# humanoid-path-planner/hpp-fcl

Hardware: AMD Instinct MI355X
Metric: narrow-phase queries/s (collision+distance) (higher is better)
Workload: dtype f32; 1 GPU; cfg3_convex32_distance_nesterov; request=distance, gather=none

## Files before the change

### hpp-fcl_amd/csrc/hfcl_dev.hpp

```cpp
#pragma once
#include <hip/hip_runtime.h>

#include <cstdint>
#include <cstring>
#include <type_traits>

#include "../../include/hppfcl_amd.h"
#include "hfcl_bvh.hpp"
#include "hfcl_bvh_shape.hpp"
#include "hfcl_pair.hpp"

using namespace hfcl;

#ifndef HFCL_WPE_GJK_W2
#define HFCL_WPE_GJK_W2 2
#endif
#ifndef HFCL_WPE_GJK
#define HFCL_WPE_GJK 3
#endif
#ifndef HFCL_WPE_GJK64
#define HFCL_WPE_GJK64 2
#endif
#ifndef HFCL_WPE_PRIM
#define HFCL_WPE_PRIM 2
#endif
#ifndef HFCL_WPE_EPA32
#define HFCL_WPE_EPA32 2
#endif
#ifndef HFCL_WPE_EPA64
#define HFCL_WPE_EPA64 1
#endif
#ifndef HFCL_WPE_BVH
#define HFCL_WPE_BVH 1
#endif

enum { B_CLOSED = 0, B_PRIM = 1, B_CC = 2, B_PC = 3, B_CP = 4, B_BVH = 5, B_UNSUPPORTED = 6, B_LARGE = 7, B_BVHSHAPE = 8, B_TRI = 9, B_COUNT = 10 };
constexpr int B_CURVED0 = B_COUNT + 4;
constexpr int CTR_SHAPE_TICKET = 2 * B_COUNT + 4, CTR_SHAPE_DEFER = 2 * B_COUNT + 5;
constexpr int CTR_DIST_SUSP = 2 * B_COUNT + 6;
constexpr int CTR_SHAPE_DIST_SUSP = 2 * B_COUNT + 7;
constexpr int CTR_DIST_TICKET = 2 * B_COUNT + 8;
constexpr int CTR_SHAPE_DIST_TICKET = 2 * B_COUNT + 9;
constexpr int CTR_EPA_CC_OVER = 2 * B_COUNT + 10;
constexpr int CTR_SHAPE_FINISH_OVER = 2 * B_COUNT + 11;
constexpr int CTR_SHAPE_DEFER_MARK = 2 * B_COUNT + 13;
constexpr int CTR_DIST_RERUN = 2 * B_COUNT + 14, CTR_SHAPE_DIST_RERUN = 2 * B_COUNT + 15;
constexpr int N_COUNTERS = 2 * B_COUNT + 16;

constexpr int K_CONVEX_LARGE = 21;

__host__ __device__ inline int bucket_of(int k1, int k2, bool distance_mode = false) {
  if (distance_mode && (k1 == K_TRIANGLE || k2 == K_TRIANGLE)) return B_UNSUPPORTED;
  const bool large = (k1 == K_CONVEX_LARGE) || (k2 == K_CONVEX_LARGE);
  if (k1 == K_CONVEX_LARGE) k1 = K_CONVEX;
  if (k2 == K_CONVEX_LARGE) k2 = K_CONVEX;
  if ((k1 == K_BVH) != (k2 == K_BVH)) {
    const int o = (k1 == K_BVH) ? k2 : k1;
    return (kind_is_prim(o) || o == K_CONVEX || kind_is_flat(o)) ? B_BVHSHAPE : B_UNSUPPORTED;
  }
  if ((k1 == K_TRIANGLE || k2 == K_TRIANGLE) && !kind_is_flat(k1) && !kind_is_flat(k2)) {
    const int o = (k1 == K_TRIANGLE) ? k2 : k1;
    return (o == K_TRIANGLE || kind_is_prim(o) || o == K_CONVEX) ? B_TRI : B_UNSUPPORTED;
  }
  const int c = pair_class(k1, k2);
  if (large && c == CLS_CONVEX) return B_LARGE;
  if (c == CLS_CLOSED) return B_CLOSED;
  if (c == CLS_PRIM_GJK) return B_PRIM;
  if (c == CLS_BVH) return B_BVH;
  if (c == CLS_CONVEX) {
    if (k1 == K_CONVEX && k2 == K_CONVEX) return B_CC;
    return (k1 == K_CONVEX) ? B_CP : B_PC;
  }
  return B_UNSUPPORTED;
}

template <typename T>
struct NbrEntry;
template <> struct alignas(16) NbrEntry<float> { float x, y, z; uint32_t id; };
template <> struct alignas(32) NbrEntry<double> { double x, y, z; uint32_t id; uint32_t pad_; };

template <typename T>
struct LibView {
  const DShape<T>* shapes;
  const T* verts;
  const uint8_t* kinds;
  uint32_t n_shapes;
  const uint32_t* graph_base;
  const uint32_t* graph_off;
  const NbrEntry<T>* graph_ent;
  uint32_t climb_min;
};
static constexpr uint32_t HFCL_NO_GRAPH = 0xFFFFFFFFu;
#ifndef HFCL_CLIMB_MIN
#define HFCL_CLIMB_MIN 512u
#endif
static constexpr int HFCL_WARM_STARTS = 14;
template <typename T>
struct HullGraph {
  const uint32_t* off;
  const NbrEntry<T>* ent;
};
template <typename T>
__device__ __forceinline__ HullGraph<T> hull_graph(const LibView<T>& lib, uint32_t shape_id, uint32_t num_points) {
  HullGraph<T> g{nullptr, nullptr};
  if (lib.graph_base == nullptr || num_points < lib.climb_min) return g;
  const uint32_t base = lib.graph_base[shape_id];
  if (base == HFCL_NO_GRAPH) return g;
  g.off = lib.graph_off + base;
  g.ent = lib.graph_ent;
  return g;
}

template <typename T> struct IO;
template <> struct IO<double> {
  const double* tf1;
  const double* tf2;
  hfcl_result* out;
  const hfcl_guess* gin;
  hfcl_guess* gout;
};
template <> struct IO<float> {
  const float* tf1;
  const float* tf2;
  hfcl_result_f32* out;
  const hfcl_guess* gin;
  hfcl_guess* gout;
};

template <typename T> using EpaItem = EpaSeed<T>;

struct Work {
  const uint32_t* shape1;
  const uint32_t* shape2;
  uint32_t n;
  uint32_t* lists;
  uint32_t* counts;
  void* epa_queue;
  void* epa_queue2;
  void* epa_v0;
  void* epa_resume;
  uint32_t resume_cap;
  void* shape_defer;
  uint32_t shape_defer_cap;
  uint32_t* shape_finish_over;
  void* shape_oq;
  void* epa_ready;
  void* epa_ready_g;
  uint32_t* epa_cc_over;
  uint32_t cc_resume_base, cc_resume_cap;
};
__host__ __device__ inline bool curved_pair(int k1, int k2) {
  return k1 == K_ELLIPSOID || k1 == K_CONE || k1 == K_CYLINDER || k2 == K_ELLIPSOID || k2 == K_CONE || k2 == K_CYLINDER;
}
struct BucketList {
  const uint32_t* base;
  uint32_t n, c0, cnt;
  __device__ __forceinline__ uint32_t operator[](uint32_t i) const { return i < c0 ? base[i] : base[n - 1u - (i - c0)]; }
};
__device__ __forceinline__ BucketList bucket_list(const Work& wk, int b) {
  const uint32_t c0 = wk.counts[b];
  return BucketList{wk.lists + size_t(b) * wk.n, wk.n, c0, c0 + wk.counts[B_CURVED0 + b]};
}
constexpr int32_t EPA_RESUME_FLAG = 0x100;
constexpr int32_t EPA_RESUME_SMALL = 0x200;

__device__ __forceinline__ Pose<double> load_pose(const double* base, uint32_t i) { return pose_from_abi<double>(base + 12 * size_t(i)); }
__device__ __forceinline__ void put_record(hfcl_result* dst, const hfcl_result& r) { *dst = r; }
__device__ __forceinline__ Pose<float> load_pose(const float* base, uint32_t i) { return pose_from_quat<float>(base + 7 * size_t(i)); }

__device__ __forceinline__ void store_record(const IO<double>& io, uint32_t pair, const PairOut<double>& o, bool contact,
                                             int nc) {
  hfcl_result r;
  r.distance = o.distance;
  r.normal[0] = o.normal.x; r.normal[1] = o.normal.y; r.normal[2] = o.normal.z;
  r.p1[0] = o.p1.x; r.p1[1] = o.p1.y; r.p1[2] = o.p1.z;
  r.p2[0] = o.p2.x; r.p2[1] = o.p2.y; r.p2[2] = o.p2.z;
  r.b1 = -1;
  r.b2 = -1;
  r.status = pack_status(o.gjk_status, o.epa_status, contact, o.gjk_iters, o.epa_iters);
  r.num_contacts = nc;
  put_record(&io.out[pair], r);
}
__device__ __forceinline__ void store_record(const IO<float>& io, uint32_t pair, const PairOut<float>& o, bool contact,
                                             int) {
  hfcl_result_f32 r;
  r.distance = o.distance;
  r.p1[0] = o.p1.x; r.p1[1] = o.p1.y; r.p1[2] = o.p1.z;
  r.p2[0] = o.p2.x; r.p2[1] = o.p2.y; r.p2[2] = o.p2.z;
  r.normal[0] = o.normal.x; r.normal[1] = o.normal.y; r.normal[2] = o.normal.z;
  r.status = pack_status(o.gjk_status, o.epa_status, contact, o.gjk_iters, o.epa_iters);
  io.out[pair] = r;
}
template <typename T>
__device__ __forceinline__ void write_out(const IO<T>& io, const QParams<T>& q, uint32_t pair, PairOut<T> o) {
  int nc;
  const bool contact = apply_query_semantics(q, o, nc);
  store_record(io, pair, o, contact, nc);
}

__device__ __forceinline__ void store_bvh_record(const IO<double>& io, uint32_t pair, const PairOut<double>& o, uint32_t nc,
                                                 int b1, int b2, bool overflow) {
  hfcl_result r;
  r.distance = o.distance;
  r.normal[0] = o.normal.x; r.normal[1] = o.normal.y; r.normal[2] = o.normal.z;
  r.p1[0] = o.p1.x; r.p1[1] = o.p1.y; r.p1[2] = o.p1.z;
  r.p2[0] = o.p2.x; r.p2[1] = o.p2.y; r.p2[2] = o.p2.z;
  r.b1 = b1;
  r.b2 = b2;
  r.status = (nc ? 128u : 0u) | (overflow ? 0xC0000000u : 0u);
  r.num_contacts = int(nc & 0x7FFFFFFFu);
  io.out[pair] = r;
}
__device__ __forceinline__ void store_bvh_record(const IO<float>& io, uint32_t pair, const PairOut<float>& o, uint32_t nc,
                                                 int, int, bool overflow) {
  hfcl_result_f32 r;
  r.distance = o.distance;
  r.p1[0] = o.p1.x; r.p1[1] = o.p1.y; r.p1[2] = o.p1.z;
  r.p2[0] = o.p2.x; r.p2[1] = o.p2.y; r.p2[2] = o.p2.z;
  r.normal[0] = o.normal.x; r.normal[1] = o.normal.y; r.normal[2] = o.normal.z;
  r.status = (nc ? 128u : 0u) | (overflow ? 0xC0000000u : 0u);
  io.out[pair] = r;
}

__device__ __forceinline__ void store_witness(const IO<double>& io, uint32_t pair, const V3<double>& p1, const V3<double>& p2, const V3<double>& n) {
  hfcl_result* r = &io.out[pair];
  r->normal[0] = n.x; r->normal[1] = n.y; r->normal[2] = n.z;
  r->p1[0] = p1.x; r->p1[1] = p1.y; r->p1[2] = p1.z;
  r->p2[0] = p2.x; r->p2[1] = p2.y; r->p2[2] = p2.z;
}
__device__ __forceinline__ void store_witness(const IO<float>& io, uint32_t pair, const V3<float>& p1, const V3<float>& p2, const V3<float>& n) {
  hfcl_result_f32* r = &io.out[pair];
  r->p1[0] = p1.x; r->p1[1] = p1.y; r->p1[2] = p1.z;
  r->p2[0] = p2.x; r->p2[1] = p2.y; r->p2[2] = p2.z;
// ... 504 lines not shown
```

### hpp-fcl_amd/csrc/hfcl_host.hip

```cpp
#include <algorithm>
#include <chrono>
#include <cstdio>
#include <cstdlib>
#include <cstring>
#include <condition_variable>
#include <map>
#include <mutex>
#include <thread>
#include <string>
#include <vector>

#include "hfcl_dev.hpp"
#include "hfcl_launch.hpp"
#include "hfcl_patch.hpp"
#include "hfcl_scene.hpp"

static thread_local std::string g_last_error;
static void set_error(const std::string& s) { g_last_error = s; }
void hfcl_internal_set_error(const char* msg) { g_last_error = msg ? msg : ""; }

#define HIP_TRY(expr)                                                                         \
  do {                                                                                        \
    hipError_t _e = (expr);                                                                   \
    if (_e != hipSuccess) {                                                                   \
      set_error(std::string(#expr) + ": " + hipGetErrorString(_e));                           \
      return HFCL_ERR_HIP;                                                                    \
    }                                                                                         \
  } while (0)

struct KernelTime {
  const char* name;
  hipEvent_t e0, e1;
  bool used;
};

struct hfcl_lib {
  int device = 0;
  size_t n_shapes = 0;
  std::vector<hfcl_shape> h_shapes;
  std::vector<uint8_t> h_kinds;
  DShape<double>* d_shapes64 = nullptr;
  DShape<float>* d_shapes32 = nullptr;
  double* d_verts64 = nullptr;
  float* d_verts32 = nullptr;
  uint8_t* d_kinds = nullptr;
  std::vector<double> h_verts;
  struct HostGraph { std::vector<uint32_t> off, ids; };
  std::map<uint32_t, HostGraph> h_graphs;
  bool graph_dirty = false;
  uint32_t* d_graph_base = nullptr;
  std::vector<void*> graph_retired;
  hipStream_t upload_stream = nullptr;
  uint32_t* d_graph_off = nullptr;
  NbrEntry<float>* d_graph_ent32 = nullptr;
  NbrEntry<double>* d_graph_ent64 = nullptr;
  uint32_t climb_min = HFCL_CLIMB_MIN;
  size_t ws_capacity = 0;
  size_t epa_capacity = 0;
  uint32_t* d_lists = nullptr;
  uint32_t* d_counts = nullptr;
  void* d_epa_queue = nullptr;
  void* d_epa_queue2 = nullptr;
  uint32_t* d_epa_cc_over = nullptr;
  hipStream_t aux = nullptr;
  hipStream_t mesh_st = nullptr;
  hipEvent_t ev_mesh_fork = nullptr, ev_mesh_join = nullptr;
  hipStream_t mesh_st2 = nullptr, mesh_aux = nullptr;
  bool ran_batch = false;
  hipEvent_t ev_mesh_fork2 = nullptr, ev_mesh_join2 = nullptr;
  BvhTask* d_bvh2_tasks = nullptr;
  void* d_bvh2_sums = nullptr;
  uint32_t* d_bvh2_susp = nullptr;
  uint32_t* d_bvh2_ctr = nullptr;
  size_t bvh2_split_n = 0, bvh2_split_cap = 0;
  uint32_t mesh_beside = 2;
  bool mesh_prio = false;
  hipStream_t gjk_st[3] = {nullptr, nullptr, nullptr};
  hipEvent_t gjk_fork = nullptr, gjk_join[3] = {nullptr, nullptr, nullptr};
  uint32_t epa_direct_max = 4096;
  uint32_t gjk_beside_max = 120000;
  hipStream_t walk_st[WALK_ROUNDS - 1] = {};
  hipEvent_t walk_fork[WALK_ROUNDS - 1] = {}, walk_join[WALK_ROUNDS - 1] = {};
  hipEvent_t ev_aux0 = nullptr, ev_aux1 = nullptr, ev_aux2 = nullptr, ev_aux3 = nullptr;
  void* d_epa_ready = nullptr;
  size_t epa_ready_capacity = 0;
  void* d_epa_ready_g = nullptr;
  size_t epa_ready_g_bytes = 0;
  bool epa_general_staged = false;
  size_t epa_general_staged_min = 32768;
  bool records_aside = true;
  bool epa64_two_streams = true;
  bool epa_cc_staged = true;
  size_t epa_cc_staged_min = 32768;
  void* d_epa_resume = nullptr;
  void* d_epa_v0 = nullptr;
  size_t resume_cap = 0;
  bool shape_finish_tiers = true;
  bool shape_finish_aside = true;
  void* d_shape_defer = nullptr;
  void* d_shape_oq = nullptr;
  size_t shape_defer_capacity = 0, shape_oq_capacity = 0;
  bool bvh_shape_lane = true;
  uint32_t shape_budget0 = 128, shape_budget = 96, shape_leaf_cost = 32, shape_levels = BVH_MAX_LEVELS;
  bool shape_coop = true;
  uint32_t bvh_cut_ticks = 0, shape_cut_ticks = 350000;
  uint32_t shape_budget0_coop = 16;
  bool bvh_coop = true;
  uint32_t bvh_budget0_coop = 0;
  uint32_t bvhd_budget = 64;
  uint32_t bvhd_pool = 1;
  uint32_t bvhd_pool_leaf_min = 24, bvhd_pool_starve = 32, bvhd_pool_part_min = 48;
  void* d_dist_susp = nullptr;
  size_t dist_susp_capacity = 0;
  uint32_t pool_rerun = 1;
  uint32_t shape_dist_pool = 1;
  uint32_t shape_dist_leaf_min = 48, shape_dist_starve = 16;
  uint32_t shape_dist_budget = 64;
  void* d_shape_dist_susp = nullptr;
  size_t shape_dist_susp_capacity = 0;
  static constexpr int PIPE_SLOTS = 6;
  struct Staging {
    uint32_t *d_s1 = nullptr, *d_s2 = nullptr;
    double *d_tf1 = nullptr, *d_tf2 = nullptr;
    double *d_qt1 = nullptr, *d_qt2 = nullptr;
    hfcl_result* d_out = nullptr;
    hfcl_guess *d_gin = nullptr, *d_gout = nullptr;
    hipEvent_t ev_in = nullptr, ev_in2 = nullptr, ev_done = nullptr;
    uint32_t* h_counts = nullptr;
    uint32_t* h_counts2 = nullptr;
    bool split = false;
  };
  Staging stage[PIPE_SLOTS];
  size_t st_capacity = 0;
  static constexpr size_t SMALL_MAX = 4096;
  char* h_pack = nullptr;
  char* d_pack = nullptr;
  uint32_t* h_pack_counts = nullptr;
  hipStream_t s_h2d = nullptr, s_h2d2 = nullptr, s_cmp = nullptr, s_d2h = nullptr;
  uint32_t acc_counts[N_COUNTERS] = {0};
  bool last_host = false;
  bool in_host_batch = false;
  size_t pipe_chunk = 0;
  uint32_t* counts_dst = nullptr;
  std::vector<KernelTime> timers;
  int split = 0;
  hfcl_lib* helper = nullptr;
  bool is_helper = false;
  bool last_split = false;
  hipStream_t side = nullptr;
  hipEvent_t ev_fork = nullptr, ev_join = nullptr;
  bool kernel_timing = true;
// ... 220 lines not shown
  lib->graph_dirty = true;
  std::vector<DShape<double>> s64(n_shapes);
  std::vector<DShape<float>> s32(n_shapes);
  std::vector<uint8_t> kinds(n_shapes);
  for (size_t i = 0; i < n_shapes; ++i) {
    const hfcl_shape& s = shapes[i];
    s64[i].kind = s.type;
    s64[i].num_points = s.num_points;
    s64[i].vertex_offset = s.vertex_offset;
    s64[i].bvh_index = s.bvh_index;
    s64[i].p0 = s.params[0];
    s64[i].p1 = s.params[1];
    s64[i].p2 = s.params[2];
    s64[i].p3 = s.params[3];
    s64[i].ssr = s.swept_sphere_radius;
    s32[i].kind = s.type;
    s32[i].num_points = s.num_points;
    s32[i].vertex_offset = s.vertex_offset;
    s32[i].bvh_index = s.bvh_index;
    s32[i].p0 = float(s.params[0]);
    s32[i].p1 = float(s.params[1]);
    s32[i].p2 = float(s.params[2]);
    s32[i].p3 = float(s.params[3]);
    s32[i].ssr = float(s.swept_sphere_radius);
    if (s.type == HFCL_GEOM_CONVEX && s.num_points > 0 && vertices &&
        size_t(s.vertex_offset) + s.num_points <= n_vertices) {
      double mn[3], mx[3];
      const double* v = vertices + 3 * size_t(s.vertex_offset);
      for (int k = 0; k < 3; ++k) mn[k] = mx[k] = v[k];
      for (uint32_t j = 1; j < s.num_points; ++j)
        for (int k = 0; k < 3; ++k) {
          mn[k] = std::min(mn[k], v[3 * size_t(j) + k]);
          mx[k] = std::max(mx[k], v[3 * size_t(j) + k]);
        }
      s64[i].p0 = (mn[0] + mx[0]) * 0.5; s64[i].p1 = (mn[1] + mx[1]) * 0.5; s64[i].p2 = (mn[2] + mx[2]) * 0.5;
      s32[i].p0 = float(s64[i].p0); s32[i].p1 = float(s64[i].p1); s32[i].p2 = float(s64[i].p2);
    }
    kinds[i] = uint8_t(s.type == HFCL_GEOM_CONVEX && s.num_points > (uint32_t)HULL_MAX ? K_CONVEX_LARGE : s.type);
  }
  {
    bool present[256] = {false};
    for (size_t i = 0; i < n_shapes; ++i) present[kinds[i]] = true;
    uint32_t mask = 1u << B_UNSUPPORTED;
    for (int a = 0; a < 256; ++a)
      if (present[a])
        for (int b = 0; b < 256; ++b)
          if (present[b]) mask |= 1u << bucket_of(a, b);
    lib->possible_buckets = mask;
    lib->has_curved = present[K_ELLIPSOID] || present[K_CONE] || present[K_CYLINDER];
    lib->has_flats = present[K_PLANE] || present[K_HALFSPACE];
  }
  lib->h_kinds = kinds;
  std::vector<float> v32(3 * n_vertices + 3);
  for (size_t i = 0; i < 3 * n_vertices; ++i) v32[i] = float(vertices[i]);
  hipFree(lib->d_shapes64); hipFree(lib->d_shapes32); hipFree(lib->d_kinds); hipFree(lib->d_verts64); hipFree(lib->d_verts32);
  lib->d_shapes64 = nullptr; lib->d_shapes32 = nullptr; lib->d_kinds = nullptr; lib->d_verts64 = nullptr; lib->d_verts32 = nullptr;
  bool ok = true;
  ok = ok && hipMalloc(&lib->d_shapes64, n_shapes * sizeof(DShape<double>)) == hipSuccess;
  ok = ok && hipMalloc(&lib->d_shapes32, n_shapes * sizeof(DShape<float>)) == hipSuccess;
  ok = ok && hipMalloc(&lib->d_kinds, n_shapes) == hipSuccess;
  ok = ok && hipMalloc(&lib->d_verts64, (3 * n_vertices + 3) * sizeof(double)) == hipSuccess;
  ok = ok && hipMalloc(&lib->d_verts32, (3 * n_vertices + 3) * sizeof(float)) == hipSuccess;
  if (ok) {
    ok = ok && hipMemcpy(lib->d_shapes64, s64.data(), n_shapes * sizeof(DShape<double>), hipMemcpyHostToDevice) == hipSuccess;
    ok = ok && hipMemcpy(lib->d_shapes32, s32.data(), n_shapes * sizeof(DShape<float>), hipMemcpyHostToDevice) == hipSuccess;
    ok = ok && hipMemcpy(lib->d_kinds, kinds.data(), n_shapes, hipMemcpyHostToDevice) == hipSuccess;
    if (n_vertices) {
      ok = ok && hipMemcpy(lib->d_verts64, vertices, 3 * n_vertices * sizeof(double), hipMemcpyHostToDevice) == hipSuccess;
      ok = ok && hipMemcpy(lib->d_verts32, v32.data(), 3 * n_vertices * sizeof(float), hipMemcpyHostToDevice) == hipSuccess;
    }
  }
  return ok;
}


static const char* const* option_keys() {
  static const char* const keys[] = {
      "closed_staged", "split", "epa_cc_staged", "epa_records_aside", "epa_general_staged", "shape_finish_tiers", "shape_finish_aside",
      "epa_general_staged_min", "epa64_two_streams", "epa_cc_staged_min", "pipe_chunk", "bvh_filter", "bvh_shape_lane", "shape_coop",
      "bvh_cut_ticks", "shape_cut_ticks", "bvh_coop", "bvhd_budget", "bvhd_pool", "shape_dist_pool", "pool_rerun", "bvh_walk_early_coop",
      "bvh_walk_rounds", "bvh_walk_order", "mesh_beside", "mesh_prio", "shape_walk", "shape_walk_sort", "shape_walk_budget", "shape_walk_min", "gjk_beside_max", "epa_direct_max", "bvh_walk_k", "bvh_walk_budget", "shape_dist_leaf_min", "shape_dist_starve", "bvhd_leaf_min", "bvhd_starve",
      "bvhd_part_min", "shape_dist_budget", "bvh_budget0_coop", "shape_budget0", "shape_budget", "shape_leaf_cost", "shape_levels",
      "climb_min", "bvh_budget", "bvh_budget0", "bvh_levels", "cvx_w", "epa_resume_slots", "bvh_task_slots", "bvh_force_wide",
      "pipe_trace", "scene_chunk", nullptr};
  return keys;
}
static int parse_list(const char* v, uint32_t* out, int first, int cap, uint32_t lo, uint32_t hi) {
  int k = first;
  for (const char* p = v; *p && k < cap; ++k) {
    const long long x = atoll(p);
    out[k] = uint32_t(std::min<long long>(std::max<long long>(x, lo), hi));
    while (*p && *p != ',') ++p;
    if (*p == ',') ++p;
  }
  return k - first;
}
static int apply_option(hfcl_lib* lib, const std::string& key, const char* v) {
  const long long i = atoll(v);
  const bool on = i != 0;
  auto u32 = [&](long long lo) { return uint32_t(std::min<long long>(std::max(i, lo), 0xFFFFFFFFll)); };
  if (key == "closed_staged") lib->closed_staged = on;
  else if (key == "split") lib->split = i >= 2 ? 2 : (i == 1 ? 1 : 0);
  else if (key == "epa_cc_staged") lib->epa_cc_staged = on;
  else if (key == "epa_records_aside") lib->records_aside = on;
  else if (key == "epa_general_staged") {
    if (on && !HFCL_KEEP_AB_FORMS) return HFCL_ERR_INVALID_ARGUMENT;
    lib->epa_general_staged = on;
  }
  else if (key == "shape_finish_tiers") lib->shape_finish_tiers = on;
  else if (key == "shape_finish_aside") lib->shape_finish_aside = on;
  else if (key == "epa_general_staged_min") lib->epa_general_staged_min = size_t(std::max(0ll, i));
  else if (key == "epa64_two_streams") lib->epa64_two_streams = on;
  else if (key == "epa_cc_staged_min") lib->epa_cc_staged_min = size_t(std::max(0ll, i));
  else if (key == "pipe_chunk") lib->pipe_chunk = strtoull(v, nullptr, 10);
  else if (key == "bvh_filter") {
    if (on && !HFCL_KEEP_AB_FORMS) return HFCL_ERR_INVALID_ARGUMENT;
    lib->bvh_filter = on;
  }
  else if (key == "bvh_shape_lane") lib->bvh_shape_lane = on;
  else if (key == "shape_coop") lib->shape_coop = on;
  else if (key == "bvh_cut_ticks") lib->bvh_cut_ticks = uint32_t(strtoul(v, nullptr, 10));
  else if (key == "shape_cut_ticks") lib->shape_cut_ticks = uint32_t(strtoul(v, nullptr, 10));
  else if (key == "bvh_coop") lib->bvh_coop = on;
  else if (key == "bvhd_budget") lib->bvhd_budget = u32(0);
  else if (key == "bvhd_pool") lib->bvhd_pool = u32(0);
  else if (key == "shape_dist_pool") lib->shape_dist_pool = u32(0);
  else if (key == "pool_rerun") lib->pool_rerun = u32(0);
  else if (key == "bvh_walk_early_coop") lib->walk_early_coop = on;
  else if (key == "bvh_walk_order") lib->walk_order = on;
  else if (key == "mesh_beside") lib->mesh_beside = u32(0);
  else if (key == "shape_walk") lib->shape_walk = on;
  else if (key == "mesh_prio") lib->mesh_prio = on;
  else if (key == "shape_walk_sort") lib->shape_walk_sort = on;
  else if (key == "shape_walk_budget") lib->shape_walk_budget = u32(0);
  else if (key == "shape_walk_min") lib->shape_walk_min = u32(0);
  else if (key == "gjk_beside_max") lib->gjk_beside_max = u32(0);
  else if (key == "epa_direct_max") lib->epa_direct_max = u32(0);
  else if (key == "bvh_walk_rounds") { lib->walk_rounds = uint32_t(std::min<long long>(std::max(0ll, i), WALK_ROUNDS)); lib->walk_auto = false; }
  else if (key == "bvh_walk_k") { parse_list(v, lib->walk_k, 0, WALK_ROUNDS, 1u, uint32_t(WALK_K)); lib->walk_auto = false; }
  else if (key == "bvh_walk_budget") parse_list(v, lib->walk_budget, 1, WALK_ROUNDS, 0u, 0xFFFFFFFFu);
  else if (key == "shape_dist_leaf_min") lib->shape_dist_leaf_min = u32(1);
  else if (key == "shape_dist_starve") lib->shape_dist_starve = u32(1);
  else if (key == "bvhd_leaf_min") lib->bvhd_pool_leaf_min = u32(1);
  else if (key == "bvhd_starve") lib->bvhd_pool_starve = u32(1);
  else if (key == "bvhd_part_min") lib->bvhd_pool_part_min = u32(0);
  else if (key == "shape_dist_budget") lib->shape_dist_budget = u32(0);
  else if (key == "bvh_budget0_coop") lib->bvh_budget0_coop = u32(1);
  else if (key == "shape_budget0") lib->shape_budget0 = lib->shape_budget0_coop = uint32_t(i);
  else if (key == "shape_budget") lib->shape_budget = uint32_t(i);
  else if (key == "shape_leaf_cost") lib->shape_leaf_cost = u32(1);
  else if (key == "shape_levels") lib->shape_levels = uint32_t(std::min<long long>(std::max(1ll, i), BVH_MAX_LEVELS));
  else if (key == "climb_min") lib->climb_min = u32(0);
  else if (key == "bvh_budget") { lib->bvh_budget = lib->bvh_budget0 = u32(0); lib->bvh_auto = false; }
  else if (key == "bvh_budget0") { lib->bvh_budget0 = u32(0); lib->bvh_auto = false; }
  else if (key == "bvh_levels") { lib->bvh_levels = uint32_t(std::min<long long>(BVH_MAX_LEVELS, std::max(1ll, i))); lib->bvh_auto = false; }
  else if (key == "cvx_w") {
    if (i == 0 || i == 2 || i == 4 || i == 8 || i == 16 || i == 32 || i == 64) lib->cvx_w = int(i);
    else return HFCL_ERR_INVALID_ARGUMENT;
  }
  else if (key == "epa_resume_slots") lib->epa_resume_slots = size_t(std::max(0ll, i));
  else if (key == "bvh_task_slots") lib->bvh_task_slots = size_t(std::max(0ll, i));
  else if (key == "bvh_force_wide") lib->bvh_force_wide = on;
  else if (key == "pipe_trace") lib->pipe_trace = on;
  else if (key == "scene_chunk") {
    if (i < 0 || i > 0xFFFFFFF0ll) return HFCL_ERR_INVALID_ARGUMENT;
    lib->scene_chunk = size_t(i);
  }
  else return HFCL_ERR_INVALID_ARGUMENT;
  return HFCL_OK;
}

hfcl_lib* hfcl_lib_create(const hfcl_shape* shapes, size_t n_shapes, const double* vertices, size_t n_vertices,
                          int device) {
  if (ensure_device(device) != HFCL_OK) return nullptr;
  if (!validate_shapes("hfcl_lib_create", shapes, n_shapes, vertices, n_vertices)) return nullptr;
  hfcl_lib* lib = new hfcl_lib();
  lib->device = device;
  bool ok = upload_shapes(lib, shapes, n_shapes, vertices, n_vertices);
  ok = ok && hipMalloc(&lib->d_counts, N_COUNTERS * sizeof(uint32_t)) == hipSuccess;
  ok = ok && hipHostMalloc((void**)&lib->h_counts, N_COUNTERS * sizeof(uint32_t), hipHostMallocDefault) == hipSuccess;
  if (ok) memset(lib->h_counts, 0, N_COUNTERS * sizeof(uint32_t));
  if (!ok) {
    set_error("hfcl_lib_create: HIP allocation/copy failed");
    hfcl_lib_destroy(lib);
    return nullptr;
  }
  hipDeviceProp_t prop;
  if (hipGetDeviceProperties(&prop, device) == hipSuccess) lib->n_cus = prop.multiProcessorCount;
  if (hipMalloc(&lib->d_epa_v0, size_t(lib->n_cus) * 16 * (64 / EPA_WE2) * EPA_MAX_VERTS * sizeof(Quad<double>)) != hipSuccess) {
    set_error("hfcl_lib_create: HIP allocation failed");
    hfcl_lib_destroy(lib);
    return nullptr;
  }
  for (const char* const* k = option_keys(); *k; ++k) {
    std::string name = "HFCL_";
    for (const char* c = *k; *c; ++c) name.push_back(char(toupper(static_cast<unsigned char>(*c))));
    if (const char* v = getenv(name.c_str())) apply_option(lib, *k, v);
  }
  return lib;
}

void hfcl_lib_destroy(hfcl_lib* lib) {
  if (!lib) return;
  hipSetDevice(lib->device);
  hipDeviceSynchronize();
  if (lib->helper) hfcl_lib_destroy(lib->helper);
  if (!lib->is_helper) free_retired_graphs(lib);
  if (lib->upload_stream) hipStreamDestroy(lib->upload_stream);
  if (lib->side) hipStreamDestroy(lib->side);
  if (lib->ev_fork) hipEventDestroy(lib->ev_fork);
  if (lib->ev_join) hipEventDestroy(lib->ev_join);
  if (!lib->is_helper) {
    hipFree(lib->d_shapes64);
    hipFree(lib->d_shapes32);
    hipFree(lib->d_kinds);
    hipFree(lib->d_verts64);
    hipFree(lib->d_verts32);
    hipFree(lib->d_graph_base);
    hipFree(lib->d_graph_off);
    hipFree(lib->d_graph_ent32);
    hipFree(lib->d_graph_ent64);
  }
  hipFree(lib->d_counts);
  if (lib->h_counts) hipHostFree(lib->h_counts);
  hipFree(lib->d_patch_ws);
  hipFree(lib->d_patch_lists);
  hipFree(lib->d_patch_counts);
  if (lib->patch_st) hipStreamDestroy(lib->patch_st);
  {
    hfcl_lib::SceneWs& w = lib->scene;
    hipFree(w.d_s1); hipFree(w.d_s2); hipFree(w.d_tf1); hipFree(w.d_tf2); hipFree(w.d_gin); hipFree(w.d_partials); hipFree(w.d_table); hipFree(w.d_summary);
    for (int k = 0; k < 2; ++k) {
      hipFree(w.d_rec[k]);
      hipFree(w.d_gout[k]);
      if (w.ev_done[k]) hipEventDestroy(w.ev_done[k]);
      if (w.ev_copied[k]) hipEventDestroy(w.ev_copied[k]);
    }
    if (w.s_cmp) hipStreamDestroy(w.s_cmp);
    if (w.s_copy) hipStreamDestroy(w.s_copy);
    if (w.h_counts) hipHostFree(w.h_counts);
    for (hipEvent_t e : w.ev_counts)
      if (e) hipEventDestroy(e);
  }
  hipFree(lib->d_lists);
  hipFree(lib->d_epa_queue);
  hipFree(lib->d_epa_queue2);
  hipFree(lib->d_epa_ready);
  hipFree(lib->d_epa_ready_g);
  hipFree(lib->d_epa_cc_over);
  if (lib->mesh_st) hipStreamDestroy(lib->mesh_st);
  if (lib->mesh_st2) hipStreamDestroy(lib->mesh_st2);
  if (lib->mesh_aux) hipStreamDestroy(lib->mesh_aux);
  for (hipEvent_t e : {lib->ev_mesh_fork, lib->ev_mesh_join, lib->ev_mesh_fork2, lib->ev_mesh_join2})
    if (e) hipEventDestroy(e);
  hipFree(lib->d_bvh2_tasks); hipFree(lib->d_bvh2_sums); hipFree(lib->d_bvh2_susp); hipFree(lib->d_bvh2_ctr);
  for (int k = 0; k < 3; ++k) {
    if (lib->gjk_st[k]) hipStreamDestroy(lib->gjk_st[k]);
    if (lib->gjk_join[k]) hipEventDestroy(lib->gjk_join[k]);
  }
  if (lib->gjk_fork) hipEventDestroy(lib->gjk_fork);
  for (int k = 0; k < WALK_ROUNDS - 1; ++k) {
    if (lib->walk_st[k]) hipStreamDestroy(lib->walk_st[k]);
    if (lib->walk_fork[k]) hipEventDestroy(lib->walk_fork[k]);
    if (lib->walk_join[k]) hipEventDestroy(lib->walk_join[k]);
  }
  if (lib->aux) hipStreamDestroy(lib->aux);
  if (lib->ev_aux0) hipEventDestroy(lib->ev_aux0);
  if (lib->ev_aux1) hipEventDestroy(lib->ev_aux1);
  if (lib->ev_aux2) hipEventDestroy(lib->ev_aux2);
  if (lib->ev_aux3) hipEventDestroy(lib->ev_aux3);
  hipFree(lib->d_epa_resume);
  hipFree(lib->d_epa_v0);
  hipFree(lib->d_shape_defer);
  hipFree(lib->d_shape_oq);
  hipFree(lib->d_dist_susp);
  hipFree(lib->d_shape_dist_susp);
  if (lib->h_pack) hipHostFree(lib->h_pack);
  if (lib->h_pack_counts) hipHostFree(lib->h_pack_counts);
  hipFree(lib->d_pack);
  for (auto& sg : lib->stage) {
    hipFree(sg.d_s1);
    hipFree(sg.d_s2);
    hipFree(sg.d_tf1);
    hipFree(sg.d_tf2);
    hipFree(sg.d_qt1);
    hipFree(sg.d_qt2);
    hipFree(sg.d_out);
    hipFree(sg.d_gin);
    hipFree(sg.d_gout);
    if (sg.ev_in) hipEventDestroy(sg.ev_in);
    if (sg.ev_done) hipEventDestroy(sg.ev_done);
    if (sg.ev_in2) hipEventDestroy(sg.ev_in2);
    if (sg.h_counts) hipHostFree(sg.h_counts);
    if (sg.h_counts2) hipHostFree(sg.h_counts2);
  }
  if (lib->s_h2d) hipStreamDestroy(lib->s_h2d);
  if (lib->s_h2d2) hipStreamDestroy(lib->s_h2d2);
  if (lib->s_cmp) hipStreamDestroy(lib->s_cmp);
  if (lib->s_d2h) hipStreamDestroy(lib->s_d2h);
  hipFree(lib->d_nodes64);
  hipFree(lib->d_nodes32);
  hipFree(lib->d_fnodes);
  hipFree(lib->d_rss64);
  hipFree(lib->d_rss32);
  hipFree(lib->d_dnodes64);
  hipFree(lib->d_dnodes32);
// ... 552 lines not shown
  for (int k = 0; k < 3; ++k) {
    lib->gjk_st[k] = s[k];
    lib->gjk_join[k] = ev[k];
  }
  lib->gjk_fork = ev[3];
  return HFCL_OK;
}
template <typename T, int M>
static int auto_cvx_w() {
  return (sizeof(T) == 8 && M == 0) ? 4 : 2;
}
template <typename T, int M>
static void launch_cvx_m(hfcl_lib* lib, const Work& wk, const LibView<T>& lv, const IO<T>& io, const QParams<T>& q,
                         hipStream_t st, size_t n) {
  const int w = lib->cvx_w ? lib->cvx_w : auto_cvx_w<T, M>();
  size_t b = (n + size_t(256 / w) - 1) / size_t(256 / w);
  if (b < 1) b = 1;
  if (b > size_t(lib->n_cus) * 16) b = size_t(lib->n_cus) * 16;
  launch_gjk_cvx<T>(M, w, q.guess_mode == HFCL_GUESS_BOUNDING_VOLUME, int(b), st, wk, lv, io, q);
}
template <typename T, class Next>
static void launch_cvx(hfcl_lib* lib, const Work& wk, const LibView<T>& lv, const IO<T>& io, const QParams<T>& q,
                       hipStream_t st, size_t& ti, size_t n, Next&& next_stream) {
  KernelTime* t = nullptr;
  auto tbeg = [&](const char* name) {
    if (!lib->kernel_timing) return;
    t = timer_slot(lib, ti++, name);
    hipEventRecord(t->e0, st);
  };
  auto tend = [&]() {
    if (lib->kernel_timing) hipEventRecord(t->e1, st);
  };
  if ((lib->possible_buckets >> B_CC) & 1u) {
    st = next_stream();
    tbeg("k_gjk_cvx<cc>");
    launch_cvx_m<T, 0>(lib, wk, lv, io, q, st, n);
    tend();
  }
  if ((lib->possible_buckets >> B_PC) & 1u) {
    st = next_stream();
    tbeg("k_gjk_cvx<pc>");
    launch_cvx_m<T, 1>(lib, wk, lv, io, q, st, n);
    tend();
  }
  if ((lib->possible_buckets >> B_CP) & 1u) {
    st = next_stream();
    tbeg("k_gjk_cvx<cp>");
    launch_cvx_m<T, 2>(lib, wk, lv, io, q, st, n);
    tend();
  }
}

template <typename T>
static int run_batch_one(hfcl_lib* lib, const uint32_t* d_s1, const uint32_t* d_s2, IO<T> io, size_t n, QParams<T> q,
                         hipStream_t st) {
  if (n == 0) return HFCL_OK;
  if (n > 0xFFFFFFF0ull) {
    set_error("batch too large (max 2^32-16 pairs per call)");
    return HFCL_ERR_LIMIT;
  }
  HIP_TRY(hipSetDevice(lib->device));
  const bool any_gjk_bucket = ((lib->possible_buckets >> B_PRIM) | (lib->possible_buckets >> B_CC) | (lib->possible_buckets >> B_PC) |
                               (lib->possible_buckets >> B_CP) | (lib->possible_buckets >> B_LARGE)) & 1u;
  int rc = ensure_workspace(lib, n, any_gjk_bucket && q.compute_penetration);
  if (rc) return rc;
  Work wk;
  wk.shape1 = d_s1;
  wk.shape2 = d_s2;
  wk.n = uint32_t(n);
  wk.lists = lib->d_lists;
  wk.counts = lib->d_counts;
  wk.epa_queue = lib->d_epa_queue;
  wk.epa_queue2 = lib->d_epa_queue2;
  wk.epa_resume = lib->d_epa_resume;
  wk.epa_v0 = lib->d_epa_v0;
  wk.resume_cap = uint32_t(std::min<size_t>(lib->resume_cap, 0xFFFFFFFFu));
  wk.shape_defer = nullptr;
  wk.shape_defer_cap = 0;
  wk.shape_finish_over = nullptr;
  wk.shape_oq = nullptr;
  wk.epa_ready = nullptr;
  wk.epa_ready_g = nullptr;
  wk.epa_cc_over = lib->d_epa_cc_over;
  wk.cc_resume_base = wk.resume_cap;
  {
    const size_t fslots = lib->resume_cap * std::max(epa_resume_stride<double>, epa_resume_stride<float>) / epa_resume_stride<float>;
    wk.cc_resume_cap = std::is_same<T, float>::value && fslots > lib->resume_cap ? uint32_t(std::min<size_t>(fslots - lib->resume_cap, lib->resume_cap)) : 0u;
  }
  LibView<T> lv;
  lv.shapes = std::is_same<T, double>::value ? (const DShape<T>*)lib->d_shapes64 : (const DShape<T>*)lib->d_shapes32;
  lv.verts = std::is_same<T, double>::value ? (const T*)lib->d_verts64 : (const T*)lib->d_verts32;
  lv.kinds = lib->d_kinds;
  lv.n_shapes = uint32_t(lib->n_shapes);
  lv.graph_base = lib->d_graph_base;
  lv.graph_off = lib->d_graph_off;
  lv.graph_ent = std::is_same<T, double>::value ? (const NbrEntry<T>*)lib->d_graph_ent64 : (const NbrEntry<T>*)lib->d_graph_ent32;
  lv.climb_min = lib->climb_min;

  for (auto& t : lib->timers) t.used = false;
  size_t ti = 0;
  const int max_blocks = lib->n_cus * 16;
  auto blocks_for = [&](size_t items, size_t per_block) {
    size_t b = (items + per_block - 1) / per_block;
    if (b < 1) b = 1;
    if (b > (size_t)max_blocks) b = max_blocks;
    return int(b);
  };
  KernelTime* t = nullptr;
  auto tbeg = [&](const char* name) {
    if (!lib->kernel_timing) return;
    t = timer_slot(lib, ti++, name);
    hipEventRecord(t->e0, st);
  };
  auto tend = [&]() {
    if (lib->kernel_timing) hipEventRecord(t->e1, st);
  };
  auto may = [&](int b) { return (lib->possible_buckets >> b) & 1u; };
  const bool any_gjk = may(B_PRIM) || may(B_CC) || may(B_PC) || may(B_CP) || may(B_LARGE);
  const bool bvg = q.guess_mode == HFCL_GUESS_BOUNDING_VOLUME;
  HIP_TRY(hipMemsetAsync(lib->d_counts, 0, N_COUNTERS * sizeof(uint32_t), st));
  tbeg("k_classify");
  launch_classify(blocks_for(n, CLS_BLOCK * 8), st, wk, lib->d_kinds, uint32_t(lib->n_shapes), q.mode != 1);
  tend();

  auto launch_solids = [&]() -> int {
    int kernels = 0;
    for (int b : {int(B_PRIM), int(B_CC), int(B_PC), int(B_CP), int(B_LARGE), int(B_TRI)}) kernels += may(b) ? 1 : 0;
    bool fan = lib->gjk_beside_max && n <= lib->gjk_beside_max && lib->h_meshes.empty() && kernels >= 3;
    if (fan && ensure_gjk_streams(lib) != HFCL_OK) fan = false;
    hipStream_t const caller = st;
    int fan_i = 0;
    uint32_t used = 0;
    if (fan) HIP_TRY(hipEventRecord(lib->gjk_fork, caller));
    auto next_stream = [&]() -> hipStream_t {
      if (!fan) return caller;
      const int k = fan_i;
      fan_i = (fan_i + 1) % 4;
      if (k && !(used & (1u << (k - 1)))) {
        used |= 1u << (k - 1);
        (void)hipStreamWaitEvent(lib->gjk_st[k - 1], lib->gjk_fork, 0);
      }
      return k ? lib->gjk_st[k - 1] : caller;
    };
    if (may(B_CLOSED)) {
      st = next_stream();
      tbeg("k_closed");
      launch_closed<T>(blocks_for(n, 256), st, wk, lv, io, q, lib->closed_staged);
      tend();
    }
    if (may(B_PRIM)) {
      st = next_stream();
      tbeg("k_gjk_prim");
      launch_gjk_prim<T>(blocks_for(n, 256), st, wk, lv, io, q, bvg);
      tend();
    }

    launch_cvx<T>(lib, wk, lv, io, q, caller, ti, n, next_stream);

    if (may(B_LARGE)) {
      st = next_stream();
      tbeg("k_gjk_large");
      launch_gjk_large<T>(blocks_for(n, 256 / LARGE_W), st, wk, lv, io, q, bvg);
      tend();
    }

    if (may(B_TRI)) {
      st = next_stream();
      tbeg("k_triangle");
      launch_triangle<T>(blocks_for(n / 8 + 1, 64 / BS_W), st, wk, lv, io, q);
      tend();
    }
    st = caller;
    for (int k = 0; k < 3; ++k)
      if (used & (1u << k)) {
        HIP_TRY(hipEventRecord(lib->gjk_join[k], lib->gjk_st[k]));
        HIP_TRY(hipStreamWaitEvent(caller, lib->gjk_join[k], 0));
      }
    return HFCL_OK;
  };
  bool meshes_on_own_stream = false;
  auto launch_meshes = [&]() -> int {
    if (!lib->h_meshes.empty() && (may(B_BVH) || may(B_BVHSHAPE))) {
      const hfcl_lib* owner = lib;
      for (const hfcl_shape& sh : owner->h_shapes)
        if (sh.type == HFCL_BV_OBBRSS && (sh.bvh_index < 0 || size_t(sh.bvh_index) >= owner->h_meshes.size())) {
          set_error("BVH shape with bvh_index " + std::to_string(sh.bvh_index) + " but only " + std::to_string(owner->h_meshes.size()) +
                    " BVHModel(s) registered (hfcl_lib_add_bvh)");
          return HFCL_ERR_INVALID_ARGUMENT;
        }
      rc = upload_bvh(lib);
      if (rc) return rc;
      BvhView<T> bv;
      bv.nodes = std::is_same<T, double>::value ? (const DNode<T>*)lib->d_nodes64 : (const DNode<T>*)lib->d_nodes32;
      bv.fnodes = (std::is_same<T, double>::value && lib->bvh_filter) ? lib->d_fnodes : nullptr;
      bv.rss = std::is_same<T, double>::value ? (const DRss<T>*)lib->d_rss64 : (const DRss<T>*)lib->d_rss32;
      bv.dnodes = std::is_same<T, double>::value ? (const DNodeD<T>*)lib->d_dnodes64 : (const DNodeD<T>*)lib->d_dnodes32;
      bv.verts = std::is_same<T, double>::value ? (const T*)lib->d_bverts64 : (const T*)lib->d_bverts32;
      bv.tris = lib->d_btris;
      bv.meshes = lib->d_meshes;
      bv.n_meshes = uint32_t(lib->h_meshes.size());
      BvhSpill spill;
      rc = make_bvh_spill(lib, spill, q.mode != 1);
      if (rc) return rc;
      auto make_split = [&](BvhSplit& split, bool want, bool solid, bool own_tables = false) -> int {
        memset(&split, 0, sizeof(split));
        split.leaf_cost = lib->shape_leaf_cost;
        if (!(want && (solid ? lib->shape_levels : lib->bvh_levels) > 1 && lib->bvh_params.num_max_contacts == 1 && !lib->bvh_params.contacts)) return HFCL_OK;
        int r = own_tables ? ensure_bvh_split2(lib, n) : ensure_bvh_split(lib, n);
        if (r) return r;
        HIP_TRY(hipMemsetAsync(own_tables ? lib->d_bvh2_ctr : lib->d_bvh_ctr, 0, BVH_CTR_WORDS * sizeof(uint32_t), st));
        split.tasks = own_tables ? lib->d_bvh2_tasks : lib->d_bvh_tasks;
        split.sums = own_tables ? lib->d_bvh2_sums : lib->d_bvh_sums;
        split.suspended = own_tables ? lib->d_bvh2_susp : lib->d_bvh_susp;
        split.ctr = own_tables ? lib->d_bvh2_ctr : lib->d_bvh_ctr;
        split.cap = uint32_t(std::min<size_t>(own_tables ? lib->bvh2_split_cap : lib->bvh_split_cap, 0x7FFFFFFFu));
        split.n_queries = uint32_t(own_tables ? lib->bvh2_split_n : lib->bvh_split_n);
        split.budget = lib->bvh_budget;
        split.budget0 = lib->bvh_budget0;
        split.n_levels = lib->bvh_levels;
        if (lib->bvh_auto && 2 * n <= 3 * size_t(lib->n_cus) * 512) {
          split.budget0 = 512;
          split.budget = 16;
          split.n_levels = BVH_MAX_LEVELS;
        }
        split.coop_grid = uint32_t(lib->n_cus) * 8u;
        split.cut_ticks = solid ? lib->shape_cut_ticks : (own_tables ? 0u : lib->bvh_cut_ticks);
        split.cut_cap = split.cap;
        split.cut_task_cap = solid ? (wk.shape_defer_cap > n ? uint32_t(std::min<size_t>(wk.shape_defer_cap - n, split.cap)) : 0u) : split.cap;
        split.cut_words = lib->d_bvh_cut_words;
        split.cut_vals = lib->d_bvh_cut_vals;
        if (!solid && lib->bvh_coop) {
          split.coop = 1u;
          const bool one_round = lib->walk_auto && n <= 220000;
          const uint32_t rounds = lib->walk_auto ? (one_round ? 1u : 2u) : lib->walk_rounds;
          split.budget0 = lib->bvh_budget0_coop ? lib->bvh_budget0_coop
                                                : (n > 500000 ? 640u : (one_round ? (n > 120000 ? 320u : 256u) : (rounds ? (n > 150000 ? std::max(320u, lib->walk_budget[0]) : lib->walk_budget[0]) : 256u)));
          if (rounds && n < (size_t(1) << 28)) {
            r = ensure_walk(lib, n);
            if (r) return r;
            HIP_TRY(hipMemsetAsync(lib->d_walk_ctr, 0, 8 * WALK_ROUNDS * sizeof(uint32_t), st));
            split.walk.recs = lib->d_walk_recs;
            split.walk.items = lib->d_walk_items;
            split.walk.res = lib->d_walk_res;
            split.walk.ctr = lib->d_walk_ctr;
            split.walk.list_in = lib->d_walk_lists;
            split.walk.list_out = lib->d_walk_lists;
            split.walk.item_cap = uint32_t(std::min<size_t>(lib->walk_n * WALK_K, 0xFFFFFFFFu));
            split.walk.list_stride = uint32_t(lib->walk_n);
            split.order = lib->walk_order ? lib->d_walk_order : nullptr;
            split.walk_rounds = std::min<uint32_t>(rounds, WALK_ROUNDS);
            for (int k = 0; k < WALK_ROUNDS; ++k) {
              split.walk_k[k] = (one_round && k == 0) ? uint32_t(WALK_K) : lib->walk_k[k];
              split.walk_budget[k] = k == 0 ? split.budget0 : lib->walk_budget[k];
            }
          }
        }
        if (solid) {
          split.coop = lib->shape_coop ? 1u : 0u;
          split.budget0 = lib->shape_coop ? lib->shape_budget0_coop : lib->shape_budget0;
          split.budget = lib->shape_budget;
          split.n_levels = lib->shape_levels;
          if (split.coop && lib->shape_walk && n >= lib->shape_walk_min && n < (size_t(1) << 28)) {
            r = ensure_swalk(lib, n);
// ... 86 lines not shown
          BvhSplit split;
          rc = make_split(split, n >= 256 && q.guess_mode != HFCL_GUESS_CACHED && !io.gout, true);
          if (rc) return rc;
          AsideStream aside = {nullptr, nullptr, nullptr};
          if (lib->shape_finish_aside && wk.shape_finish_over && split.tasks && split.coop && split.cut_ticks) {
            rc = ensure_aux(lib);
            if (rc) return rc;
            aside = AsideStream{meshes_on_own_stream ? lib->mesh_aux : lib->aux, lib->ev_aux2, lib->ev_aux3};
          }
          launch_bvh_shape_fast<T>(blocks_for(n, BVH_BLOCK), blocks_for(n / 8 + 1, 64 / BS_W), int(std::min<size_t>(n / 4 + 1, size_t(lib->n_cus) * 8)), st, wk, lv, bv, io, q, lib->bvh_params,
                                   T(lib->break_distance * lib->break_distance), split, spill, aside.stream ? &aside : nullptr);
        } else {
          launch_bvh_shape<T>(blocks_for(n / 8 + 1, 64 / BS_W), st, wk, lv, bv, io, q, lib->bvh_params, T(lib->break_distance * lib->break_distance));
        }
        tend();
        if (mm_beside) {
          HIP_TRY(hipStreamWaitEvent(st, lib->ev_mesh_join2, 0));
        } else {
          rc = mesh_mesh(false);
          if (rc) return rc;
        }
      } else {
        tbeg("k_bvh_shape_distance");
        if (shape_fast_d) {
          BvhSpill ss;
          memset(&ss, 0, sizeof(ss));
          if (lib->shape_dist_budget && q.guess_mode != HFCL_GUESS_CACHED && !io.gout) {
            if (lib->ws_capacity > lib->shape_dist_susp_capacity) {
              hipFree(lib->d_shape_dist_susp);
              lib->d_shape_dist_susp = nullptr;
              lib->shape_dist_susp_capacity = 0;
              HIP_TRY(hipMalloc(&lib->d_shape_dist_susp, lib->ws_capacity * sizeof(ShapeDistSusp<double>)));
              lib->shape_dist_susp_capacity = lib->ws_capacity;
            }
            ss.susp = lib->d_shape_dist_susp;
            ss.rerun_count = lib->pool_rerun ? lib->d_counts + CTR_SHAPE_DIST_RERUN : nullptr;
            ss.rerun_all = lib->pool_rerun >= 2 ? 1u : 0u;
            ss.susp_count = lib->d_counts + CTR_SHAPE_DIST_SUSP;
            ss.budget = lib->shape_dist_budget;
            ss.max_blocks = uint32_t(lib->n_cus) * 8u;
            ss.pool = lib->has_flats ? 0u : lib->shape_dist_pool;
            ss.pool_ticket = lib->d_counts + CTR_SHAPE_DIST_TICKET;
            ss.pool_leaf_min = lib->shape_dist_leaf_min;
            ss.pool_starve = lib->shape_dist_starve;
          }
          launch_bvh_shape_distance_fast<T>(blocks_for(n, BVHD_BLOCK), blocks_for(n / 8 + 1, 64 / BS_W), st, wk, lv, bv, io, q, ss);
        }
        else
          launch_bvh_shape_distance<T>(blocks_for(n / 8 + 1, 64 / BS_W), st, wk, lv, bv, io, q);
        tend();
        tbeg("k_bvh_distance");
        if (may(B_BVH) && !spill.wide && lib->bvhd_budget) {
          if (lib->ws_capacity > lib->dist_susp_capacity) {
            hipFree(lib->d_dist_susp);
            lib->d_dist_susp = nullptr;
            lib->dist_susp_capacity = 0;
            HIP_TRY(hipMalloc(&lib->d_dist_susp, lib->ws_capacity * sizeof(DistSusp<double>)));
            lib->dist_susp_capacity = lib->ws_capacity;
          }
          spill.susp = lib->d_dist_susp;
          spill.rerun_count = lib->pool_rerun ? lib->d_counts + CTR_DIST_RERUN : nullptr;
          spill.rerun_all = lib->pool_rerun >= 2 ? 1u : 0u;
          spill.susp_count = lib->d_counts + CTR_DIST_SUSP;
          spill.budget = lib->bvhd_budget;
          spill.max_blocks = uint32_t(lib->n_cus) * 8u;
          spill.pool = lib->bvhd_pool;
          spill.pool_ticket = lib->d_counts + CTR_DIST_TICKET;
          spill.pool_leaf_min = lib->bvhd_pool_leaf_min;
          spill.pool_starve = lib->bvhd_pool_starve;
          spill.pool_part_min = lib->bvhd_pool_part_min;
          if (lib->bvh_max_nodes > 32767) spill.pool = 0;
        }
        launch_bvh_distance<T>(blocks_for(n, BVHD_BLOCK), st, wk, lv, bv, io, q, spill);
        tend();
      }
    }
    return HFCL_OK;
  };
  bool mesh_join_pending = false;
  {
    const bool any_mesh = !lib->h_meshes.empty() && (may(B_BVH) || may(B_BVHSHAPE));
    const bool any_solid = may(B_CLOSED) || any_gjk || may(B_TRI);
    bool beside = any_mesh && any_solid && lib->mesh_beside;
    if (beside && lib->mesh_beside < 4 && lib->ran_batch && lib->h_counts) {
      uint32_t solids_before = 0, meshes_before = one_count(lib->h_counts, int(B_BVH)) + one_count(lib->h_counts, int(B_BVHSHAPE));
      for (int b : {int(B_CLOSED), int(B_PRIM), int(B_CC), int(B_PC), int(B_CP), int(B_LARGE), int(B_TRI)}) solids_before += one_count(lib->h_counts, b);
      if (!solids_before || !meshes_before) beside = false;
    }
    if (beside && ensure_mesh_stream(lib) != HFCL_OK) beside = false;
    if (beside) {
      hipStream_t const caller = st;
      HIP_TRY(hipEventRecord(lib->ev_mesh_fork, caller));
      HIP_TRY(hipStreamWaitEvent(lib->mesh_st, lib->ev_mesh_fork, 0));
      st = lib->mesh_st;
      meshes_on_own_stream = true;
      rc = launch_meshes();
      st = caller;
      if (rc) return rc;
      HIP_TRY(hipEventRecord(lib->ev_mesh_join, lib->mesh_st));
      rc = launch_solids();
      if (rc) return rc;
      if (lib->mesh_beside < 2) HIP_TRY(hipStreamWaitEvent(caller, lib->ev_mesh_join, 0));
      else mesh_join_pending = true;
    } else {
      rc = launch_solids();
      if (rc) return rc;
      rc = launch_meshes();
      if (rc) return rc;
    }
  }

  if (q.compute_penetration && any_gjk) {
    constexpr bool F32 = std::is_same<T, float>::value;
    const bool general_q = may(B_PRIM) || may(B_PC) || may(B_CP) || (!F32 && may(B_CC));
    bool cc_staged = false;
    if constexpr (F32) cc_staged = may(B_CC) && lib->epa_cc_staged && n >= lib->epa_cc_staged_min;
    bool gen_staged = general_q && lib->epa_general_staged && n >= lib->epa_general_staged_min;
    const bool direct = sizeof(T) == 8 && lib->epa_direct_max && n <= lib->epa_direct_max;
    auto need_aux = [&]() -> int { return ensure_aux(lib); };
    auto tbeg_on = [&](const char* name, hipStream_t s) {
      if (!lib->kernel_timing) return;
      t = timer_slot(lib, ti++, name);
      hipEventRecord(t->e0, s);
    };
    auto tend_on = [&](hipStream_t s) {
      if (lib->kernel_timing) hipEventRecord(t->e1, s);
    };
    if (direct) cc_staged = gen_staged = false;
    if (cc_staged) {
      if (lib->ws_capacity > lib->epa_ready_capacity) {
        hipFree(lib->d_epa_ready);
        lib->d_epa_ready = nullptr;
        lib->epa_ready_capacity = 0;
        HIP_TRY(hipMalloc(&lib->d_epa_ready, lib->ws_capacity * sizeof(EpaReady<float>)));
        lib->epa_ready_capacity = lib->ws_capacity;
      }
      wk.epa_ready = lib->d_epa_ready;
    }
    if (gen_staged) {
      if (lib->ws_capacity * sizeof(EpaReadyG<T>) > lib->epa_ready_g_bytes) {
        hipFree(lib->d_epa_ready_g);
        lib->d_epa_ready_g = nullptr;
        lib->epa_ready_g_bytes = 0;
        HIP_TRY(hipMalloc(&lib->d_epa_ready_g, lib->ws_capacity * sizeof(EpaReadyG<T>)));
        lib->epa_ready_g_bytes = lib->ws_capacity * sizeof(EpaReadyG<T>);
      }
      wk.epa_ready_g = lib->d_epa_ready_g;
    }
    if constexpr (F32) {
      if (cc_staged) {
        tbeg("k_epa_prepare");
        launch_epa_prepare(blocks_for(n / 4 + 1, 256), st, wk, lv, io, q);
        tend();
      }
    }
    if (gen_staged) {
      tbeg("k_epa_prepare_general");
      launch_epa_prepare_general<T>(blocks_for(n / 4 + 1, 256), st, wk, lv, io, q, F32);
      tend();
    }
    if (direct) {
      tbeg("k_epa<full>");
      launch_epa_requeue<T>(st, wk);
      launch_epa_full<T>(int(std::min<size_t>(blocks_for(n / 2 + 1, 64 / epa_we2<T>), size_t(lib->n_cus) * 16)), st, wk, lv, io, q);
      tend();
    } else {
    const int epa_batches = int(std::min<size_t>((n + 64 / EPA_WE - 1) / (64 / EPA_WE), size_t(1) << 22));
    tbeg("k_epa<fast>");
    hipStream_t st2 = nullptr;
    if constexpr (!F32) {
      if (lib->epa64_two_streams && lib->has_curved && general_q) {
        if (int rc2 = need_aux()) return rc2;
        st2 = lib->aux;
        HIP_TRY(hipEventRecord(lib->ev_aux0, st));
        HIP_TRY(hipStreamWaitEvent(st2, lib->ev_aux0, 0));
      }
    }
    if constexpr (F32) {
      if (cc_staged) launch_epa_loop(epa_batches, st, wk, lv, q, lib->n_cus);
    }
    if (gen_staged) launch_epa_loop_general<T>(epa_batches, st, st2, wk, lv, q, lib->n_cus, lib->has_curved);
    if ((F32 && may(B_CC) && !cc_staged) || (general_q && !gen_staged))
      launch_epa_fast<T>(epa_batches, st, wk, lv, io, q, may(B_CC) && !cc_staged, general_q && !gen_staged, lib->n_cus, lib->has_curved, st2);
    if (st2) {
      HIP_TRY(hipEventRecord(lib->ev_aux1, st2));
      HIP_TRY(hipStreamWaitEvent(st, lib->ev_aux1, 0));
    }
    tend();
    if (cc_staged || gen_staged) {
      const bool aside = lib->records_aside;
      if (aside) {
        if (int rc2 = need_aux()) return rc2;
        HIP_TRY(hipEventRecord(lib->ev_aux0, st));
        HIP_TRY(hipStreamWaitEvent(lib->aux, lib->ev_aux0, 0));
      }
      hipStream_t rs = aside ? lib->aux : st;
      tbeg_on("k_epa_records", rs);
      if constexpr (F32) {
        if (cc_staged) launch_epa_records(blocks_for(n / 4 + 1, 256), rs, wk, lv, io, q);
      }
      if (gen_staged) launch_epa_records_general<T>(blocks_for(n / 4 + 1, 256), rs, wk, lv, io, q, F32);
      tend_on(rs);
      hipStream_t fs = cc_staged ? rs : st;
      tbeg_on("k_epa<full>", fs);
      launch_epa_full<T>(blocks_for(n / 16 + 1, 64 / epa_we2<T>), fs, wk, lv, io, q);
      tend_on(fs);
      if (aside) HIP_TRY(hipEventRecord(lib->ev_aux1, rs));
      if constexpr (F32) {
        if (cc_staged) {
          tbeg("k_epa_resume_cc");
          launch_epa_resume_cc(blocks_for(n / 16 + 1, 64 / HFCL_EPA_CC_RESUME_WE), st, wk, lv, io, q);
          tend();
        }
      }
      if (aside) HIP_TRY(hipStreamWaitEvent(st, lib->ev_aux1, 0));
    } else {
      tbeg("k_epa<full>");
      launch_epa_full<T>(blocks_for(n / 16 + 1, 64 / epa_we2<T>), st, wk, lv, io, q);
      tend();
    }
    }
  }
  if (mesh_join_pending) HIP_TRY(hipStreamWaitEvent(st, lib->ev_mesh_join, 0));
  tbeg("k_unsupported");
  if (may(B_UNSUPPORTED)) launch_unsupported<T>(blocks_for(n, 256 * 64), st, wk, io, int(B_UNSUPPORTED));
  if (lib->h_meshes.empty()) {
    if (may(B_BVHSHAPE)) launch_unsupported<T>(blocks_for(n, 256 * 64), st, wk, io, int(B_BVHSHAPE));
    if (may(B_BVH)) launch_unsupported<T>(blocks_for(n, 256 * 64), st, wk, io, int(B_BVH));
  }
  tend();
  HIP_TRY(hipMemcpyAsync(lib->counts_dst ? lib->counts_dst : lib->h_counts, lib->d_counts, N_COUNTERS * sizeof(uint32_t), hipMemcpyDeviceToHost, st));
  lib->ran_batch = lib->counts_dst == nullptr;
  HIP_TRY(hipGetLastError());
  return HFCL_OK;
}

static void share_tables(hfcl_lib* h, const hfcl_lib* lib) {
  h->n_shapes = lib->n_shapes;
  h->d_shapes64 = lib->d_shapes64;
  h->d_shapes32 = lib->d_shapes32;
  h->d_verts64 = lib->d_verts64;
  h->d_verts32 = lib->d_verts32;
  h->d_kinds = lib->d_kinds;
  h->possible_buckets = lib->possible_buckets;
  h->has_curved = lib->has_curved;
  h->has_flats = lib->has_flats;
  h->d_graph_base = lib->d_graph_base;
  h->d_graph_off = lib->d_graph_off;
  h->d_graph_ent32 = lib->d_graph_ent32;
  h->d_graph_ent64 = lib->d_graph_ent64;
  h->climb_min = lib->climb_min;
}
static hfcl_lib* make_helper(hfcl_lib* lib) {
  hfcl_lib* h = new hfcl_lib;
  h->is_helper = true;
  h->device = lib->device;
  share_tables(h, lib);
  h->cvx_w = lib->cvx_w;
  h->epa_resume_slots = lib->epa_resume_slots;
  h->closed_staged = lib->closed_staged;
  h->epa_cc_staged = lib->epa_cc_staged;
  h->records_aside = lib->records_aside;
  h->epa_general_staged = lib->epa_general_staged;
  h->shape_finish_tiers = lib->shape_finish_tiers;
  h->shape_finish_aside = lib->shape_finish_aside;
  h->shape_cut_ticks = lib->shape_cut_ticks;
  h->epa_general_staged_min = lib->epa_general_staged_min;
  h->epa64_two_streams = lib->epa64_two_streams;
  h->epa_cc_staged_min = lib->epa_cc_staged_min;
  h->n_cus = lib->n_cus;
  bool ok = hipMalloc(&h->d_counts, N_COUNTERS * sizeof(uint32_t)) == hipSuccess;
  ok = ok && hipHostMalloc((void**)&h->h_counts, N_COUNTERS * sizeof(uint32_t), hipHostMallocDefault) == hipSuccess;
  ok = ok && hipMalloc(&h->d_epa_v0, size_t(h->n_cus) * 16 * (64 / EPA_WE2) * EPA_MAX_VERTS * sizeof(Quad<double>)) == hipSuccess;
  if (!ok) {
    hfcl_lib_destroy(h);
    return nullptr;
  }
  memset(h->h_counts, 0, N_COUNTERS * sizeof(uint32_t));
  return h;
}

template <typename T> static IO<T> io_at(const IO<T>& io, size_t lo);
template <> IO<double> io_at(const IO<double>& io, size_t lo) {
  return IO<double>{io.tf1 + 12 * lo, io.tf2 + 12 * lo, io.out + lo, io.gin ? io.gin + lo : nullptr, io.gout ? io.gout + lo : nullptr};
}
template <> IO<float> io_at(const IO<float>& io, size_t lo) {
  return IO<float>{io.tf1 + 7 * lo, io.tf2 + 7 * lo, io.out + lo, nullptr, nullptr};
}

static bool batch_splits(const hfcl_lib* lib, size_t n) {
  constexpr size_t MIN_SPLIT = 1u << 17;
  int parts = lib->split;
  if (parts == 0) {
    int kinds = 0;
    for (int b : {int(B_PRIM), int(B_CC), int(B_PC), int(B_CP), int(B_LARGE)}) kinds += (lib->possible_buckets >> b) & 1u;
    parts = kinds >= 3 ? 2 : 1;
  }
  return parts >= 2 && n >= MIN_SPLIT && lib->h_meshes.empty();
}
static int ensure_helper(hfcl_lib* lib) {
  if (lib->helper) return HFCL_OK;
  HIP_TRY(hipSetDevice(lib->device));
  lib->helper = make_helper(lib);
  bool ok = lib->helper != nullptr;
  ok = ok && (lib->side || hipStreamCreateWithFlags(&lib->side, hipStreamNonBlocking) == hipSuccess);
  ok = ok && (lib->ev_fork || hipEventCreateWithFlags(&lib->ev_fork, hipEventDisableTiming) == hipSuccess);
  ok = ok && (lib->ev_join || hipEventCreateWithFlags(&lib->ev_join, hipEventDisableTiming) == hipSuccess);
  if (!ok) {
    if (lib->helper) hfcl_lib_destroy(lib->helper);
    lib->helper = nullptr;
    set_error("split batches: HIP allocation failed");
    return HFCL_ERR_HIP;
  }
  return HFCL_OK;
}

template <typename T>
static int run_batch(hfcl_lib* lib, const uint32_t* d_s1, const uint32_t* d_s2, IO<T> io, size_t n, QParams<T> q,
                     hipStream_t st) {
  lib->last_split = false;
  if (!lib->in_host_batch) lib->last_host = false;
  if (lib->graph_dirty) {
    const int rcg = upload_graph(lib);
    if (rcg) return rcg;
  }
  if (!batch_splits(lib, n)) return run_batch_one<T>(lib, d_s1, d_s2, io, n, q, st);
  int rc0 = ensure_helper(lib);
  if (rc0) return rc0;
  hfcl_lib* h2 = lib->helper;
  h2->kernel_timing = lib->kernel_timing;
  h2->break_distance = lib->break_distance;
  h2->bvh_params = lib->bvh_params;
  const size_t h = n / 2;
  HIP_TRY(hipEventRecord(lib->ev_fork, st));
  HIP_TRY(hipStreamWaitEvent(lib->side, lib->ev_fork, 0));
  int rc = run_batch_one<T>(lib, d_s1, d_s2, io, h, q, st);
  if (rc) return rc;
  rc = run_batch_one<T>(h2, d_s1 + h, d_s2 + h, io_at<T>(io, h), n - h, q, lib->side);
  if (rc) return rc;
  HIP_TRY(hipEventRecord(lib->ev_join, lib->side));
  HIP_TRY(hipStreamWaitEvent(st, lib->ev_join, 0));
  lib->last_split = true;
  return HFCL_OK;
}

template <typename T>
static int setup_collide(const hfcl_collision_request* req, QParams<T>& q, bool& skip_all) {
  skip_all = false;
  if (!req) {
    set_error("null request");
    return HFCL_ERR_INVALID_ARGUMENT;
  }
  if (req->num_max_contacts == 0) {
    set_error("Invalid number of max contacts (current value is 0).");
    return HFCL_ERR_INVALID_ARGUMENT;
// ... 60 lines not shown
  int rc = setup_collide<double>(req, q, skip);
  if (rc) return rc;
  hipStream_t st = (hipStream_t)stream;
  if (skip) {
    HIP_TRY(hipSetDevice(lib->device));
    if (n) launch_fill_skipped(st, d_out, uint32_t(n));
    return HFCL_OK;
  }
  IO<double> io{d_tf1, d_tf2, d_out, d_guess_in, d_guess_out};
  lib->bvh_params.num_max_contacts = req->num_max_contacts;
  lib->break_distance = req->break_distance;
  return run_batch<double>(lib, d_shape1, d_shape2, io, n, q, st);
}

int hfcl_distance_batch_device(hfcl_lib* lib, const uint32_t* d_shape1, const uint32_t* d_shape2, const double* d_tf1,
                               const double* d_tf2, size_t n, const hfcl_distance_request* req, hfcl_result* d_out,
                               const hfcl_guess* d_guess_in, hfcl_guess* d_guess_out, void* stream) {
  if (!lib) {
    set_error("null library");
    return HFCL_ERR_INVALID_ARGUMENT;
  }
  QParams<double> q;
  int rc = setup_distance<double>(req, q);
  if (rc) return rc;
  IO<double> io{d_tf1, d_tf2, d_out, d_guess_in, d_guess_out};
  return run_batch<double>(lib, d_shape1, d_shape2, io, n, q, (hipStream_t)stream);
}

int hfcl_distance_batch_device_f32(hfcl_lib* lib, const uint32_t* d_shape1, const uint32_t* d_shape2,
                                   const float* d_pose1, const float* d_pose2, size_t n,
                                   const hfcl_distance_request* req, hfcl_result_f32* d_out, void* stream) {
  if (!lib) {
    set_error("null library");
    return HFCL_ERR_INVALID_ARGUMENT;
  }
  QParams<float> q;
  int rc = setup_distance<float>(req, q);
  if (rc) return rc;
  IO<float> io{d_pose1, d_pose2, d_out, nullptr, nullptr};
  return run_batch<float>(lib, d_shape1, d_shape2, io, n, q, (hipStream_t)stream);
}

int hfcl_collide_batch_device_f32(hfcl_lib* lib, const uint32_t* d_shape1, const uint32_t* d_shape2,
                                  const float* d_pose1, const float* d_pose2, size_t n,
                                  const hfcl_collision_request* req, hfcl_result_f32* d_out, void* stream) {
  if (!lib) {
    set_error("null library");
    return HFCL_ERR_INVALID_ARGUMENT;
  }
  QParams<float> q;
  bool skip;
  int rc = setup_collide<float>(req, q, skip);
  if (rc) return rc;
  hipStream_t st = (hipStream_t)stream;
  if (skip) {
    HIP_TRY(hipSetDevice(lib->device));
    if (n) launch_fill_skipped(st, d_out, uint32_t(n));
    return HFCL_OK;
  }
  IO<float> io{d_pose1, d_pose2, d_out, nullptr, nullptr};
  lib->bvh_params.num_max_contacts = req->num_max_contacts;
  lib->break_distance = req->break_distance;
  return run_batch<float>(lib, d_shape1, d_shape2, io, n, q, st);
}

int hfcl_compact_results_device(hfcl_lib* lib, const hfcl_result* d_records, size_t n, hfcl_result_compact* d_out, void* stream) {
  return compact_results(lib, d_records, n, d_out, stream);
}
int hfcl_compact_results_device_f32(hfcl_lib* lib, const hfcl_result_f32* d_records, size_t n, hfcl_result_compact_f32* d_out,
                                    void* stream) {
  return compact_results(lib, d_records, n, d_out, stream);
}

static int ensure_staging(hfcl_lib* lib, size_t n, bool gin, bool gout, bool compact) {
  if (!lib->s_cmp) {
    HIP_TRY(hipStreamCreateWithFlags(&lib->s_h2d, hipStreamNonBlocking));
    HIP_TRY(hipStreamCreateWithFlags(&lib->s_h2d2, hipStreamNonBlocking));
    HIP_TRY(hipStreamCreateWithFlags(&lib->s_cmp, hipStreamNonBlocking));
    HIP_TRY(hipStreamCreateWithFlags(&lib->s_d2h, hipStreamNonBlocking));
    for (auto& sg : lib->stage) {
      HIP_TRY(hipEventCreateWithFlags(&sg.ev_in, hipEventDisableTiming));
      HIP_TRY(hipEventCreateWithFlags(&sg.ev_done, hipEventDisableTiming));
      HIP_TRY(hipEventCreateWithFlags(&sg.ev_in2, hipEventDisableTiming));
      HIP_TRY(hipHostMalloc((void**)&sg.h_counts, N_COUNTERS * sizeof(uint32_t), hipHostMallocDefault));
      HIP_TRY(hipHostMalloc((void**)&sg.h_counts2, N_COUNTERS * sizeof(uint32_t), hipHostMallocDefault));
    }
  }
  if (n > lib->st_capacity) {
    lib->st_capacity = 0;
    const size_t cap = n + n / 8 + 256;
    for (auto& sg : lib->stage) {
      hipFree(sg.d_s1); hipFree(sg.d_s2); hipFree(sg.d_tf1); hipFree(sg.d_tf2); hipFree(sg.d_out);
      hipFree(sg.d_gin); hipFree(sg.d_gout); hipFree(sg.d_qt1); hipFree(sg.d_qt2);
      sg.d_qt1 = sg.d_qt2 = nullptr;
      sg.d_s1 = sg.d_s2 = nullptr;
      sg.d_tf1 = sg.d_tf2 = nullptr;
      sg.d_out = nullptr;
      sg.d_gin = sg.d_gout = nullptr;
      HIP_TRY(hipMalloc(&sg.d_s1, cap * sizeof(uint32_t)));
      HIP_TRY(hipMalloc(&sg.d_s2, cap * sizeof(uint32_t)));
      HIP_TRY(hipMalloc(&sg.d_tf1, cap * 12 * sizeof(double)));
      HIP_TRY(hipMalloc(&sg.d_tf2, cap * 12 * sizeof(double)));
      HIP_TRY(hipMalloc(&sg.d_out, cap * sizeof(hfcl_result)));
    }
    lib->st_capacity = cap;
  }
  for (auto& sg : lib->stage) {
    if (gin && !sg.d_gin) HIP_TRY(hipMalloc(&sg.d_gin, lib->st_capacity * sizeof(hfcl_guess)));
    if (gout && !sg.d_gout) HIP_TRY(hipMalloc(&sg.d_gout, lib->st_capacity * sizeof(hfcl_guess)));
    if (compact && !sg.d_qt1) {
      HIP_TRY(hipMalloc(&sg.d_qt1, lib->st_capacity * 7 * sizeof(double)));
      HIP_TRY(hipMalloc(&sg.d_qt2, lib->st_capacity * 7 * sizeof(double)));
    }
  }
  return HFCL_OK;
}

static int host_batch_checks(hfcl_lib* lib, const hfcl_collision_request* creq, const hfcl_distance_request* dreq) {
  const bool skipped = creq && creq->security_margin == -__builtin_inf();
  if (!skipped && total_count(lib, B_UNSUPPORTED) > 0) {
    set_error("Collision/distance function between some node types of the batch is not yet supported (" +
              std::to_string(total_count(lib, B_UNSUPPORTED)) + " pairs; their records carry status bit 31)");
    return HFCL_ERR_UNSUPPORTED_PAIR;
  }
  {
    const hfcl_query_request& qq = creq ? creq->q : dreq->q;
    if (!skipped && qq.gjk_initial_guess == HFCL_GUESS_BOUNDING_VOLUME &&
        (total_count(lib, B_TRI) > 0 || total_count(lib, B_BVHSHAPE) > 0)) {
      set_error("computeLocalAABB must have been called on the shapes before using GJKInitialGuess::BoundingVolumeGuess.");
      return HFCL_ERR_INVALID_ARGUMENT;
    }
  }
  if (!skipped && creq && creq->security_margin < 0 && total_count(lib, B_BVHSHAPE) > 0) {
    set_error("Negative security margin are not handled yet for BVHModel");
    return HFCL_ERR_INVALID_ARGUMENT;
  }
  if (!skipped && (total_count(lib, B_BVH) > 0 || total_count(lib, B_BVHSHAPE) > 0) && lib->h_meshes.empty()) {
    set_error("BVH shapes in the batch but no BVHModel registered (hfcl_lib_add_bvh)");
    return HFCL_ERR_INVALID_ARGUMENT;
  }
  return HFCL_OK;
}

struct SmallBatchBuckets {
  hfcl_lib* lib;
  uint32_t library_buckets;
  SmallBatchBuckets(hfcl_lib* l, const uint32_t* s1, const uint32_t* s2, size_t n, bool distance_mode) : lib(l), library_buckets(l->possible_buckets) {
    if (n > 1024 || lib->h_kinds.size() != lib->n_shapes) return;
    uint32_t mask = 0;
    for (size_t i = 0; i < n; ++i)
      mask |= 1u << ((s1[i] < lib->n_shapes && s2[i] < lib->n_shapes) ? bucket_of(lib->h_kinds[s1[i]], lib->h_kinds[s2[i]], distance_mode)
                                                                       : int(B_UNSUPPORTED));
    lib->possible_buckets = mask & (library_buckets | (1u << B_UNSUPPORTED));
    if (lib->helper) lib->helper->possible_buckets = lib->possible_buckets;
  }
  ~SmallBatchBuckets() {
    lib->possible_buckets = library_buckets;
    if (lib->helper) lib->helper->possible_buckets = library_buckets;
  }
};

static int host_batch_small(hfcl_lib* lib, const uint32_t* s1, const uint32_t* s2, const double* tf1, const double* tf2, size_t n,
                            const hfcl_collision_request* creq, const hfcl_distance_request* dreq, hfcl_result* out,
                            const hfcl_guess* gin, hfcl_guess* gout, bool compact) {
  constexpr size_t C = hfcl_lib::SMALL_MAX;
  auto up = [](size_t x) { return (x + 255) & ~size_t(255); };
  const size_t pose_in = compact ? 7 : 12;
  const size_t o_p1 = 0, o_p2 = o_p1 + n * pose_in * 8, o_gin = o_p2 + n * pose_in * 8, o_s1 = o_gin + (gin ? n * sizeof(hfcl_guess) : 0),
               o_s2 = o_s1 + up(n * 4), in_bytes = o_s2 + up(n * 4);
  const size_t o_out = up(in_bytes), o_gout = o_out + n * sizeof(hfcl_result), out_bytes = n * sizeof(hfcl_result) + (gout ? n * sizeof(hfcl_guess) : 0);
  const size_t o_tf1 = up(o_out + out_bytes), o_tf2 = o_tf1 + n * 96;
  if (!lib->d_pack) {
    const size_t cap = up(C * (2 * 96 + sizeof(hfcl_guess)) + 2 * up(C * 4)) + up(C * (sizeof(hfcl_result) + sizeof(hfcl_guess))) + 2 * C * 96 + 1024;
    HIP_TRY(hipHostMalloc((void**)&lib->h_pack, cap, hipHostMallocDefault));
    HIP_TRY(hipHostMalloc((void**)&lib->h_pack_counts, 2 * N_COUNTERS * sizeof(uint32_t), hipHostMallocDefault));
    HIP_TRY(hipMalloc(&lib->d_pack, cap));
  }
  if (!lib->s_cmp) {
    const int rc0 = ensure_staging(lib, 256, false, false, false);
    if (rc0) return rc0;
  }
  char* h = lib->h_pack;
  char* d = lib->d_pack;
  memcpy(h + o_p1, tf1, n * pose_in * 8);
  memcpy(h + o_p2, tf2, n * pose_in * 8);
  if (gin) memcpy(h + o_gin, gin, n * sizeof(hfcl_guess));
  memcpy(h + o_s1, s1, n * 4);
  memcpy(h + o_s2, s2, n * 4);
  hipStream_t st = lib->s_cmp;
  HIP_TRY(hipMemcpyAsync(d, h, in_bytes, hipMemcpyHostToDevice, st));
  const double *d_tf1 = reinterpret_cast<const double*>(d + o_p1), *d_tf2 = reinterpret_cast<const double*>(d + o_p2);
  if (compact) {
    launch_expand_poses(st, d_tf1, reinterpret_cast<double*>(d + o_tf1), uint32_t(n));
    launch_expand_poses(st, d_tf2, reinterpret_cast<double*>(d + o_tf2), uint32_t(n));
    d_tf1 = reinterpret_cast<const double*>(d + o_tf1);
    d_tf2 = reinterpret_cast<const double*>(d + o_tf2);
  }
  memset(lib->acc_counts, 0, sizeof(lib->acc_counts));
  memset(lib->h_pack_counts, 0, 2 * N_COUNTERS * sizeof(uint32_t));
  lib->in_host_batch = true;
  lib->counts_dst = lib->h_pack_counts;
  if (lib->helper) lib->helper->counts_dst = lib->h_pack_counts + N_COUNTERS;
  int rc;
  {
    SmallBatchBuckets batch_buckets(lib, s1, s2, n, dreq != nullptr);
    const uint32_t* d_s1 = reinterpret_cast<const uint32_t*>(d + o_s1);
    const uint32_t* d_s2 = reinterpret_cast<const uint32_t*>(d + o_s2);
    const hfcl_guess* d_gin = gin ? reinterpret_cast<const hfcl_guess*>(d + o_gin) : nullptr;
    hfcl_guess* d_gout = gout ? reinterpret_cast<hfcl_guess*>(d + o_gout) : nullptr;
    if (creq)
      rc = hfcl_collide_batch_device(lib, d_s1, d_s2, d_tf1, d_tf2, n, creq, reinterpret_cast<hfcl_result*>(d + o_out), d_gin, d_gout, st);
    else
      rc = hfcl_distance_batch_device(lib, d_s1, d_s2, d_tf1, d_tf2, n, dreq, reinterpret_cast<hfcl_result*>(d + o_out), d_gin, d_gout, st);
  }
  hipError_t e = hipSuccess;
  if (rc == HFCL_OK) e = hipMemcpyAsync(h + o_out, d + o_out, out_bytes, hipMemcpyDeviceToHost, st);
  const hipError_t e2 = hipStreamSynchronize(st);
  lib->in_host_batch = false;
  lib->counts_dst = nullptr;
  if (lib->helper) lib->helper->counts_dst = nullptr;
  if (rc) return rc;
  if (e != hipSuccess || e2 != hipSuccess) {
    set_error(std::string("host batch (small): ") + hipGetErrorString(e != hipSuccess ? e : e2));
    return HFCL_ERR_HIP;
  }
  memcpy(out, h + o_out, n * sizeof(hfcl_result));
  if (gout) memcpy(gout, h + o_gout, n * sizeof(hfcl_guess));
  for (int i = 0; i < N_COUNTERS; ++i) lib->acc_counts[i] = lib->h_pack_counts[i] + (lib->last_split ? lib->h_pack_counts[N_COUNTERS + i] : 0u);
  lib->last_host = true;
  return host_batch_checks(lib, creq, dreq);
}

static int host_batch(hfcl_lib* lib, const uint32_t* s1, const uint32_t* s2, const double* tf1, const double* tf2,
                      size_t n, const hfcl_collision_request* creq, const hfcl_distance_request* dreq, hfcl_result* out,
                      const hfcl_guess* gin, hfcl_guess* gout, bool pipelined = true, bool compact = false, bool f32 = false) {
  if (!lib) {
    set_error("null library");
    return HFCL_ERR_INVALID_ARGUMENT;
  }
  if (n == 0) return HFCL_OK;
  if (!s1 || !s2 || !tf1 || !tf2 || !out) {
    set_error("null buffer");
    return HFCL_ERR_INVALID_ARGUMENT;
  }
  HIP_TRY(hipSetDevice(lib->device));
  if (pipelined && n <= hfcl_lib::SMALL_MAX && !lib->pipe_chunk && !f32) return host_batch_small(lib, s1, s2, tf1, tf2, n, creq, dreq, out, gin, gout, compact);
  std::vector<size_t> bounds;
  bounds.push_back(0);
  size_t max_chunk = n;
  if (pipelined && lib->pipe_chunk) {
    for (size_t lo = 0; lo < n; lo += lib->pipe_chunk) bounds.push_back(std::min(n, lo + lib->pipe_chunk));
    max_chunk = std::min(n, lib->pipe_chunk);
  } else if (pipelined && f32 && n > (size_t(1) << 16)) {
    const size_t c = std::min<size_t>(std::max<size_t>((n + 2) / 3, size_t(1) << 16), size_t(1) << 19);
    for (size_t lo = 0; lo < n; lo += c) bounds.push_back(std::min(n, lo + c));
    max_chunk = std::min(n, c);
  } else if (pipelined && n > (size_t(1) << 16)) {
    const size_t steady = std::min<size_t>(std::max<size_t>(n / 6, size_t(1) << 16), size_t(1) << 18);
// ... 873 lines not shown
  launch_scene_expand(st, ea, f32, max_blocks);
  const int rc = scene_batch(lib, w.d_s1, w.d_s2, w.d_tf1, w.d_tf2, m, creq, dreq, d_rec, d_gin, d_gout, st);
  if (rc) return rc;
  if (d_summary) {
    SceneFoldArgs fa;
    fa.rec = d_rec;
    fa.q0 = q0;
    fa.q1 = q0 + m;
    fa.n_pairs = uint32_t(s->n_pairs);
    fa.g0 = scene_piece_of(q0, fa.n_pairs);
    fa.n_pieces = scene_piece_of(q0 + m - 1, fa.n_pairs) - fa.g0 + 1;
    fa.margin = creq ? creq->security_margin : 0.0;
    fa.collide = creq ? 1 : 0;
    fa.summary = d_summary;
    fa.partials = scene_shares(fa.n_pairs) > 1u ? w.d_partials : nullptr;
    launch_scene_fold(st, fa, f32, max_blocks);
  }
  return HFCL_OK;
}
static void scene_join_side(hfcl_lib* lib, hipStream_t st) {
  if (lib->side && lib->ev_join && hipEventRecord(lib->ev_join, lib->side) == hipSuccess) (void)hipStreamWaitEvent(st, lib->ev_join, 0);
}

template <typename T>
static int scene_device(const char* who, hfcl_scene* s, const void* d_table, size_t n_conf, const hfcl_collision_request* creq,
                        const hfcl_distance_request* dreq, typename SceneTypes<T>::R* d_out, hfcl_scene_summary* d_summary,
                        const hfcl_guess* d_gin, hfcl_guess* d_gout, hipStream_t st) {
  size_t total;
  int rc = scene_validate<T>(who, s, d_table, n_conf, creq, dreq, d_out, d_summary, total);
  if (rc || !total) return rc;
  hfcl_lib* lib = s->lib;
  HIP_TRY(hipSetDevice(lib->device));
  const size_t chunk = scene_chunk_size(lib, total);
  rc = scene_workspace(lib, chunk, d_out ? 0 : 1, false, 0, d_summary ? scene_pieces_bound(s->n_pairs, chunk) : 0);
  if (rc) return rc;
  for (size_t q0 = 0; q0 < total; q0 += chunk) {
    const size_t m = std::min(chunk, total - q0);
    auto* rec = d_out ? d_out + q0 : static_cast<typename SceneTypes<T>::R*>(lib->scene.d_rec[0]);
    rc = scene_chunk_run<T>(s, d_table, q0, m, creq, dreq, rec, d_summary, d_gin ? d_gin + q0 : nullptr, d_gout ? d_gout + q0 : nullptr, st);
    if (rc) {
      scene_join_side(lib, st);
      return rc;
    }
  }
  HIP_TRY(hipGetLastError());
  return HFCL_OK;
}

template <typename T>
static int scene_host(const char* who, hfcl_scene* s, const void* table, size_t n_conf, const hfcl_collision_request* creq,
                      const hfcl_distance_request* dreq, typename SceneTypes<T>::R* out, hfcl_scene_summary* summary, const hfcl_guess* gin,
                      hfcl_guess* gout) {
  using R = typename SceneTypes<T>::R;
  size_t total;
  int rc = scene_validate<T>(who, s, table, n_conf, creq, dreq, out, summary, total);
  if (rc || !total) return rc;
  hfcl_lib* lib = s->lib;
  hfcl_lib::SceneWs& w = lib->scene;
  HIP_TRY(hipSetDevice(lib->device));
  if (!w.s_cmp) HIP_TRY(hipStreamCreateWithFlags(&w.s_cmp, hipStreamNonBlocking));
  if (!w.s_copy) HIP_TRY(hipStreamCreateWithFlags(&w.s_copy, hipStreamNonBlocking));
  for (int k = 0; k < 2; ++k) {
    if (!w.ev_done[k]) HIP_TRY(hipEventCreateWithFlags(&w.ev_done[k], hipEventDisableTiming));
    if (!w.ev_copied[k]) HIP_TRY(hipEventCreateWithFlags(&w.ev_copied[k], hipEventDisableTiming));
  }
  const size_t chunk = scene_chunk_size(lib, total);
  const size_t n_chunks = (total + chunk - 1) / chunk;
  const bool back = out != nullptr || gout != nullptr;
  rc = scene_workspace(lib, chunk, out ? 2 : 1, gin != nullptr, gout ? 2 : 0, summary ? scene_pieces_bound(s->n_pairs, chunk) : 0);
  if (rc) return rc;
  const size_t table_bytes = n_conf * s->n_objects * SceneTypes<T>::WIDTH * sizeof(T);
  {
    char* t = static_cast<char*>(w.d_table);
    rc = scene_grow(&t, w.table_bytes, table_bytes, 1);
    w.d_table = t;
    if (rc) return rc;
  }
  if (summary) {
    rc = scene_grow(&w.d_summary, w.summary_cap, n_conf, sizeof(hfcl_scene_summary));
    if (rc) return rc;
  }
  constexpr int CS = hfcl_lib::SceneWs::COUNT_SLOTS;
  constexpr size_t SLOT_WORDS = 2 * size_t(N_COUNTERS);
  if (!w.h_counts) HIP_TRY(hipHostMalloc((void**)&w.h_counts, CS * SLOT_WORDS * sizeof(uint32_t), hipHostMallocDefault));
  for (hipEvent_t& e : w.ev_counts)
    if (!e) HIP_TRY(hipEventCreateWithFlags(&e, hipEventDisableTiming));
  memset(w.h_counts, 0, CS * SLOT_WORDS * sizeof(uint32_t));
  bool slot_split[CS] = {};
  memset(lib->acc_counts, 0, sizeof(lib->acc_counts));
  auto harvest = [&](int slot) {
    uint32_t* c = w.h_counts + size_t(slot) * SLOT_WORDS;
    for (int i = 0; i < N_COUNTERS; ++i) lib->acc_counts[i] += c[i] + (slot_split[slot] ? c[N_COUNTERS + i] : 0u);
    memset(c, 0, SLOT_WORDS * sizeof(uint32_t));
  };
  lib->in_host_batch = true;

  auto finish = [&](int code) {
    hipStreamSynchronize(w.s_cmp);
    hipStreamSynchronize(w.s_copy);
    if (lib->side) hipStreamSynchronize(lib->side);
    lib->in_host_batch = false;
    lib->counts_dst = nullptr;
    if (lib->helper) lib->helper->counts_dst = nullptr;
    return code;
  };
#define SCENE_TRY(expr)                                                      \
  do {                                                                       \
    hipError_t _e = (expr);                                                  \
    if (_e != hipSuccess) {                                                  \
      set_error(std::string(#expr) + ": " + hipGetErrorString(_e));          \
      return finish(HFCL_ERR_HIP);                                           \
    }                                                                        \
  } while (0)
  auto copy_back = [&](size_t k) -> hipError_t {
    const int b = int(k & 1);
    const size_t q0 = k * chunk, m = std::min(chunk, total - q0);
    hipError_t e = hipStreamWaitEvent(w.s_copy, w.ev_done[b], 0);
    if (e == hipSuccess && out) e = hipMemcpyAsync(out + q0, w.d_rec[b], m * sizeof(R), hipMemcpyDeviceToHost, w.s_copy);
    if (e == hipSuccess && gout) e = hipMemcpyAsync(gout + q0, w.d_gout[b], m * sizeof(hfcl_guess), hipMemcpyDeviceToHost, w.s_copy);
    if (e == hipSuccess) e = hipEventRecord(w.ev_copied[b], w.s_copy);
    return e;
  };

  SCENE_TRY(hipMemcpyAsync(w.d_table, table, table_bytes, hipMemcpyHostToDevice, w.s_cmp));
  for (size_t k = 0; k < n_chunks; ++k) {
    const int b = back ? int(k & 1) : 0;
    const size_t q0 = k * chunk, m = std::min(chunk, total - q0);
    if (back && k >= 2) SCENE_TRY(hipStreamWaitEvent(w.s_cmp, w.ev_copied[b], 0));
    if (gin) SCENE_TRY(hipMemcpyAsync(w.d_gin, gin + q0, m * sizeof(hfcl_guess), hipMemcpyHostToDevice, w.s_cmp));
    const int slot = int(k % CS);
    if (k >= size_t(CS)) {
      SCENE_TRY(hipEventSynchronize(w.ev_counts[slot]));
      harvest(slot);
    }
    lib->counts_dst = w.h_counts + size_t(slot) * SLOT_WORDS;
    if (batch_splits(lib, m)) {
      rc = ensure_helper(lib);
      if (rc) return finish(rc);
      lib->helper->counts_dst = lib->counts_dst + N_COUNTERS;
    }
    rc = scene_chunk_run<T>(s, w.d_table, q0, m, creq, dreq, static_cast<R*>(w.d_rec[out ? b : 0]), summary ? w.d_summary : nullptr,
                            gin ? w.d_gin : nullptr, gout ? w.d_gout[b] : nullptr, w.s_cmp);
    if (rc) return finish(rc);
    slot_split[slot] = lib->last_split;
    SCENE_TRY(hipEventRecord(w.ev_counts[slot], w.s_cmp));
    if (back) {
      SCENE_TRY(hipEventRecord(w.ev_done[b], w.s_cmp));
      if (k >= 1) SCENE_TRY(copy_back(k - 1));
    }
  }
  if (back) SCENE_TRY(copy_back(n_chunks - 1));
  if (summary) SCENE_TRY(hipMemcpyAsync(summary, w.d_summary, n_conf * sizeof(hfcl_scene_summary), hipMemcpyDeviceToHost, w.s_cmp));
  SCENE_TRY(hipStreamSynchronize(w.s_cmp));
  SCENE_TRY(hipStreamSynchronize(w.s_copy));
  SCENE_TRY(hipGetLastError());
#undef SCENE_TRY
  for (int slot = 0; slot < CS && size_t(slot) < n_chunks; ++slot) harvest(slot);
  lib->in_host_batch = false;
  lib->counts_dst = nullptr;
  if (lib->helper) lib->helper->counts_dst = nullptr;
  lib->last_host = true;
  return host_batch_checks(lib, creq, dreq);
}

extern "C" {

hfcl_scene* hfcl_scene_create(hfcl_lib* lib, const uint32_t* object_shape, size_t n_objects, const uint32_t* pairs, size_t n_pairs) {
// ... 116 lines not shown
```

### hpp-fcl_amd/csrc/hfcl_k_epa.hip

```cpp
#include <algorithm>

#include "hfcl_dev.hpp"
#include "hfcl_launch.hpp"

#ifndef HFCL_UNIT_PRECISION
#define HFCL_UNIT_PRECISION 0
#endif
#define HFCL_UNIT_F32 (HFCL_UNIT_PRECISION != 64)
#define HFCL_UNIT_F64 (HFCL_UNIT_PRECISION != 32)

template <typename T, int WE, bool LARGE>
struct EpaSupport {
  DShape<T> a, b;
  HullRegs<T, WE> h0, h1;
  const T* va;
  const T* vb;
  HullGraph<T> ga, gb;
  mutable int hint0, hint1;
  MDiff<T> md;
  int lig;
  __device__ __forceinline__ V3<T> hull(const DShape<T>& s, const HullRegs<T, WE>& h, const T* v, const HullGraph<T>& g, const V3<T>& d, int& hint) const {
    if (LARGE && s.num_points > uint32_t(HULL_MAX)) return large_hull_support<T, WE>(v, s.num_points, g, d, lig, hint);
    return h.support(d, lig);
  }
// ... 176 lines not shown
            const T ssr = swept_radius(lib.shapes[wk.shape1[pair]]) + swept_radius(lib.shapes[wk.shape2[pair]]);
            EpaResult<T> res;
            if constexpr (CC)
              epa.loop_result(L, ssr, res, tags_of(ip));
            else
              epa.loop_result(L, ssr, res);
            finish(res, ip);
          } else {
            uint32_t slot = 0;
            if (lig == 0) slot = atomicAdd(&wk.counts[B_COUNT + 1], 1u);
            slot = __shfl(slot, 0, WE);
            const bool save = epa.resumable && slot < wk.resume_cap;
            if (save) {
              if constexpr (CC)
                epa_save_block<T, Grp, CAP>(&scratch[grp], resume_slot<T, CAP>(wk, slot), tags_of(ip));
              else
                epa_save_block<T, Grp, CAP>(&scratch[grp], resume_slot<T, CAP>(wk, slot));
            }
            if (lig == 0) {
              EpaItem<T>* dst = reinterpret_cast<EpaItem<T>*>(wk.epa_queue2) + slot;
              *dst = *ip;
              if (save) dst->rank = ip->rank | EPA_RESUME_FLAG | (CAP != epa_fast_cap<T> ? EPA_RESUME_SMALL : 0);
            }
          }
          Grp::sync();
          state = IDLE;
        }
        const uint64_t lower = live | ~((uint64_t(1) << (grp * WE)) - 1);
        const uint32_t rank = uint32_t(__popcll(~lower)) / WE;
        it = next + rank * gridDim.x;
        if (it < cnt) {
          const EpaItem<T>* ip = item_ptr(it);
          const uint32_t pair = ip->pair;
          {
            const DShape<T> a = lib.shapes[wk.shape1[pair]], b = lib.shapes[wk.shape2[pair]];
            if (CC || a.kind == K_CONVEX) sup.h0.load(lib.verts + 3 * size_t(a.vertex_offset), a.num_points, lig);
            if (CC || b.kind == K_CONVEX) sup.h1.load(lib.verts + 3 * size_t(b.vertex_offset), b.num_points, lig);
            if constexpr (!CC) {
              sup.a = a;
              sup.b = b;
            }
            sup.md = make_mdiff(load_pose(io.tf1, pair), load_pose(io.tf2, pair));
          }
          epa.reset(&scratch[grp], q.epa_max_iterations, q.epa_tolerance);
          epa.set_vert(0, ip->w[0], ip->w0[0], -1);
          epa.set_vert(1, ip->w[1], ip->w0[1], -2);
          epa.set_vert(2, ip->w[2], ip->w0[2], -3);
          epa.set_vert(3, ip->w[3], ip->w0[3], -4);
          Grp::sync();
          EpaResult<T> res;
          int closest0;
          if constexpr (CC)
            closest0 = epa.begin(ip->rank, -ip->guess, sup, res, tags_of(ip));
          else
            closest0 = epa.begin(ip->rank, -ip->guess, sup, res);
          if (closest0 != EPA_NULL) {
            epa.loop_enter(L, closest0, 0, 0);
            state = LIVE;
          } else if (epa.overflow) {
            state = HANDOVER;
          } else {
            finish(res, ip);
          }
        }
      }
      next += uint32_t(G - n_live) * gridDim.x;
      if (n_live == 0 && !more) {
        if (__ballot(state == LIVE) == 0) break;
      }
      continue;
    }
    if (state == LIVE) {
      const int r = epa.step(L, sup);
      if (r != 0) state = r == 1 ? DONE : HANDOVER;
    }
  }
}

template <typename T>
__global__ void __launch_bounds__(256) k_epa_prepare(Work wk, LibView<T> lib, IO<T> io, QParams<T> q) {
  const uint32_t cnt = wk.counts[B_COUNT + 3];
  const EpaItem<T>* const queue = reinterpret_cast<const EpaItem<T>*>(wk.epa_queue);
  EpaReady<T>* const ready = reinterpret_cast<EpaReady<T>*>(wk.epa_ready);
  for (uint32_t i = blockIdx.x * blockDim.x + threadIdx.x; i < cnt; i += gridDim.x * blockDim.x) {
    bool live = false;
    EpaReady<T> rb;
    {
      const EpaItem<T>* ip = queue + (wk.n - 1u - i);
      const int rank = ip->rank;
      if (rank != 4) {
        const uint32_t slot = atomicAdd(&wk.counts[B_COUNT + 1], 1u);
        reinterpret_cast<EpaItem<T>*>(wk.epa_queue2)[slot] = *ip;
      } else {
        const V3<T> w[4] = {ip->w[0], ip->w[1], ip->w[2], ip->w[3]};
        int flags[4], closest = 0;
        live = epa_prepare_tetrahedron(w, q.epa_tolerance, rb.vw, rb.fn, flags, closest);
        const uint32_t pair = ip->pair;
        if (live) {
          const DShape<T> a = lib.shapes[wk.shape1[pair]], b = lib.shapes[wk.shape2[pair]];
          const MDiff<T> md = make_mdiff(load_pose(io.tf1, pair), load_pose(io.tf2, pair));
          rb.seed = i;
          rb.voff_a = a.vertex_offset;
          rb.voff_b = b.vertex_offset;
          rb.packed = (a.num_points & 63u) | ((b.num_points & 63u) << 6) | (uint32_t(closest) << 12) | (uint32_t((flags[0] >> 1) & 1) << 14) |
                      (uint32_t((flags[1] >> 1) & 1) << 15) | (uint32_t((flags[2] >> 1) & 1) << 16) | (uint32_t((flags[3] >> 1) & 1) << 17) |
                      (md.identity ? 1u << 18 : 0u);
          rb.md[0] = md.oR1.r0.x; rb.md[1] = md.oR1.r0.y; rb.md[2] = md.oR1.r0.z;
          rb.md[3] = md.oR1.r1.x; rb.md[4] = md.oR1.r1.y; rb.md[5] = md.oR1.r1.z;
          rb.md[6] = md.oR1.r2.x; rb.md[7] = md.oR1.r2.y; rb.md[8] = md.oR1.r2.z;
          rb.md[9] = md.ot1.x; rb.md[10] = md.ot1.y; rb.md[11] = md.ot1.z;
          rb.state = EPA_READY_PENDING;
          rb.pair = pair;
          rb.gjk_iters = ip->gjk_iters;
          rb.pad_ = 0u;
        } else {
          EpaResult<T> res;
          res.status = EPA_FALLBACK;
          res.iterations = 0;
          PairOut<T> o;
          epa_finish(res, ip->gjk_iters, load_pose(io.tf1, pair), T(0), T(0), o);
          write_out<T>(io, q, pair, o);
          write_guess<T>(io, pair, o.cached_guess, 0, 0);
        }
      }
    }
    if (live) {
      ready[i] = rb;
    } else {
      ready[i].packed = 0u;
      ready[i].state = EPA_READY_NONE;
    }
  }
}

#ifndef HFCL_EPA_LOOP_REFILL_MIN
#define HFCL_EPA_LOOP_REFILL_MIN 2
#endif
#ifndef HFCL_EPA_LOOP_ROUNDS
#define HFCL_EPA_LOOP_ROUNDS 1
#endif
#ifndef HFCL_EPA_CC_RESUME
#define HFCL_EPA_CC_RESUME 1
#endif
template <typename T>
__device__ __forceinline__ EpaSaved<T, EPA_FAST_CAP>* cc_resume_slot(const Work& wk, uint32_t slot) {
  return resume_slot<T, EPA_FAST_CAP>(wk, wk.cc_resume_base + slot);
}
template <typename T, int WE, int CAP>
__global__ void __launch_bounds__(64) __attribute__((amdgpu_waves_per_eu(HFCL_WPE_EPA32_CC, 8)))
k_epa_loop(Work wk, LibView<T> lib, QParams<T> q) {
  constexpr int G = 64 / WE;
  static_assert(WE >= 8, "a group's lanes copy the eight records of a block");
  typedef LaneGroup<WE> Grp;
  __shared__ EpaScratch<T, CAP, V0_TAG> scratch[G];
  const uint32_t cnt = wk.counts[B_COUNT + 3];
  const int lane = threadIdx.x & 63, grp = lane / WE, lig = lane & (WE - 1);
  EpaReady<T>* const ready = reinterpret_cast<EpaReady<T>*>(wk.epa_ready);
  const EpaItem<T>* const queue = reinterpret_cast<const EpaItem<T>*>(wk.epa_queue);
  enum { IDLE = 0, LIVE = 1, DONE = 2, HANDOVER = 3 };
  int state = IDLE;
  uint32_t it = 0;
  uint32_t next = blockIdx.x;
  EpaSupportCC<T, WE> sup;
  sup.lig = lig;
  Epa<T, Grp, CAP, V0_TAG> epa;
  EpaLoop<T> L;
  while (true) {
    const uint64_t live = __ballot(state == LIVE);
    const int n_live = __popcll(live) / WE;
    const bool more = next < cnt;
    if (n_live == 0 || (more && G - n_live >= HFCL_EPA_LOOP_REFILL_MIN)) {
      if (state != LIVE) {
        if (state != IDLE) {
          EpaReady<T>* rb = ready + it;
          if (state == DONE) {
            EpaLoopOut<T> o;
            epa.loop_out(L, o);
            if (lig == 0) {
              *reinterpret_cast<EpaLoopOut<T>*>(rb->md) = o;
              rb->state = EPA_READY_DONE;
            }
          } else {
            uint32_t slot = 0xFFFFFFFFu;
            if (HFCL_EPA_CC_RESUME && epa.resumable) {
              if (lig == 0) slot = atomicAdd(&wk.counts[CTR_EPA_CC_OVER], 1u);
              slot = __shfl(slot, 0, WE);
            }
            if (slot < wk.cc_resume_cap) {
              epa_save_block<T, Grp, CAP, V0_TAG, NoTags, true>(&scratch[grp], cc_resume_slot<T>(wk, slot));
              if (lig == 0) wk.epa_cc_over[slot] = it;
            } else {
              if (lig == 0) {
                const EpaItem<T>* ip = queue + (wk.n - 1u - rb->seed);
                const uint32_t s2 = atomicAdd(&wk.counts[B_COUNT + 1], 1u);
                reinterpret_cast<EpaItem<T>*>(wk.epa_queue2)[s2] = *ip;
              }
            }
            if (lig == 0) rb->state = EPA_READY_HANDED_OVER;
          }
          Grp::sync();
          state = IDLE;
        }
        const uint64_t lower = live | ~((uint64_t(1) << (grp * WE)) - 1);
        const uint32_t rank = uint32_t(__popcll(~lower)) / WE;
        it = next + rank * gridDim.x;
        if (it < cnt) {
          const EpaReady<T>* rb = ready + it;
          const uint32_t packed = rb->packed;
          if ((packed & 63u) != 0u) {
          sup.h0.load(lib.verts + 3 * size_t(rb->voff_a), packed & 63u, lig);
          sup.h1.load(lib.verts + 3 * size_t(rb->voff_b), (packed >> 6) & 63u, lig);
          sup.md.oR1.r0 = mk<T>(rb->md[0], rb->md[1], rb->md[2]);
          sup.md.oR1.r1 = mk<T>(rb->md[3], rb->md[4], rb->md[5]);
          sup.md.oR1.r2 = mk<T>(rb->md[6], rb->md[7], rb->md[8]);
          sup.md.ot1 = mk<T>(rb->md[9], rb->md[10], rb->md[11]);
          sup.md.identity = (packed >> 18) & 1u;
          epa.reset(&scratch[grp], q.epa_max_iterations, q.epa_tolerance);
          epa.loop_enter(L, epa.install(rb, packed), 0, 0);
          state = LIVE;
          }
        }
      }
      next += uint32_t(G - n_live) * gridDim.x;
      if (n_live == 0 && !more) {
        if (__ballot(state == LIVE) == 0) break;
      }
      continue;
    }
    if (state == LIVE) {
      const int r = epa.step(L, sup);
      if (r != 0) state = r == 1 ? DONE : HANDOVER;
    }
  }
}

template <typename T, int WE>
__global__ void __launch_bounds__(64) k_epa_resume_cc(Work wk, LibView<T> lib, IO<T> io, QParams<T> q) {
  constexpr int G = 64 / WE, CAP = EPA_MAX_ITER;
  typedef LaneGroup<WE> Grp;
  __shared__ EpaScratch<T, CAP, V0_TAG> scratch[G];
  const uint32_t cnt = min(wk.counts[CTR_EPA_CC_OVER], wk.cc_resume_cap);
  const int lane = threadIdx.x & 63, grp = lane / WE, lig = lane & (WE - 1);
  const EpaReady<T>* const ready = reinterpret_cast<const EpaReady<T>*>(wk.epa_ready);
  const EpaItem<T>* const queue = reinterpret_cast<const EpaItem<T>*>(wk.epa_queue);
  for (uint32_t it = blockIdx.x * G + grp; it < cnt; it += gridDim.x * G) {
    const uint32_t idx = wk.epa_cc_over[it];
    if (idx == 0xFFFFFFFFu) continue;
    const EpaReady<T>* rb = ready + idx;
    const uint32_t packed = rb->packed, pair = rb->pair;
    EpaSupportCC<T, WE> sup;
    sup.lig = lig;
    const T* va = lib.verts + 3 * size_t(rb->voff_a);
    sup.h0.load(va, packed & 63u, lig);
    sup.h1.load(lib.verts + 3 * size_t(rb->voff_b), (packed >> 6) & 63u, lig);
    sup.md.oR1.r0 = mk<T>(rb->md[0], rb->md[1], rb->md[2]);
    sup.md.oR1.r1 = mk<T>(rb->md[3], rb->md[4], rb->md[5]);
    sup.md.oR1.r2 = mk<T>(rb->md[6], rb->md[7], rb->md[8]);
    sup.md.ot1 = mk<T>(rb->md[9], rb->md[10], rb->md[11]);
    sup.md.identity = (packed >> 18) & 1u;
    const SeedTags<T> tags{va, queue + (wk.n - 1u - rb->seed)};
    const T r0 = swept_radius(lib.shapes[wk.shape1[pair]]), r1 = swept_radius(lib.shapes[wk.shape2[pair]]);
    Epa<T, Grp, CAP, V0_TAG> epa;
    epa.reset(&scratch[grp], q.epa_max_iterations, q.epa_tolerance);
    const EpaHeader h = epa.template load<EPA_FAST_CAP>(cc_resume_slot<T>(wk, it));
    EpaResult<T> res;
    epa.run_loop(h.closest, h.iterations, h.pass, r0 + r1, sup, res, tags);
    PairOut<T> o;
    epa_finish(res, rb->gjk_iters, load_pose(io.tf1, pair), r0, r1, o);
    if (lig == 0) {
      write_out<T>(io, q, pair, o);
      write_guess<T>(io, pair, o.cached_guess, 0, 0);
    }
    Grp::sync();
  }
}

template <typename T>
__global__ void __launch_bounds__(256) k_epa_records(Work wk, LibView<T> lib, IO<T> io, QParams<T> q) {
  const uint32_t cnt = wk.counts[B_COUNT + 3];
  const EpaReady<T>* const ready = reinterpret_cast<const EpaReady<T>*>(wk.epa_ready);
  const EpaItem<T>* const queue = reinterpret_cast<const EpaItem<T>*>(wk.epa_queue);
  for (uint32_t i = blockIdx.x * blockDim.x + threadIdx.x; i < cnt; i += gridDim.x * blockDim.x) {
    const EpaReady<T>* rb = ready + i;
    if (rb->state != EPA_READY_DONE) continue;
    const EpaLoopOut<T>* lo = reinterpret_cast<const EpaLoopOut<T>*>(rb->md);
    const uint32_t pair = rb->pair;
    const SeedTags<T> tags{lib.verts + 3 * size_t(rb->voff_a), queue + (wk.n - 1u - rb->seed)};
    const T r0 = swept_radius(lib.shapes[wk.shape1[pair]]), r1 = swept_radius(lib.shapes[wk.shape2[pair]]);
    EpaResult<T> res;
    res.status = lo->status;
    res.iterations = lo->iterations;
    res.normal = mk<T>(lo->nx, lo->ny, lo->nz);
    res.depth = lo->depth + (r0 + r1);
    res.rw0_ = mk<T>(lo->rw[0], lo->rw[1], lo->rw[2]);
    res.rw1_ = mk<T>(lo->rw[3], lo->rw[4], lo->rw[5]);
    res.rw2_ = mk<T>(lo->rw[6], lo->rw[7], lo->rw[8]);
    res.r00 = tags(lo->tag[0]);
    res.r01 = tags(lo->tag[1]);
    res.r02 = tags(lo->tag[2]);
    PairOut<T> o;
    epa_finish(res, rb->gjk_iters, load_pose(io.tf1, pair), r0, r1, o);
    write_out<T>(io, q, pair, o);
    write_guess<T>(io, pair, o.cached_guess, 0, 0);
  }
}

template <typename T>
// ... 142 lines not shown
      const int r = epa.step(L, sup);
      if (r != 0) state = r == 1 ? DONE : HANDOVER;
    }
  }
}

template <typename T>
__global__ void __launch_bounds__(256) k_epa_records_general(Work wk, LibView<T> lib, IO<T> io, QParams<T> q, int skip_top) {
  const uint32_t cnt0 = wk.counts[B_COUNT], cnt = cnt0 + (skip_top ? 0u : wk.counts[B_COUNT + 3]);
  for (uint32_t it = blockIdx.x * blockDim.x + threadIdx.x; it < cnt; it += gridDim.x * blockDim.x) {
    const bool top = it >= cnt0;
    const EpaReadyG<T>* rb = ready_g<T>(wk, top, top ? it - cnt0 : it);
    if (rb->state != EPA_READY_DONE) continue;
    const EpaLoopOutG<T>* lo = reinterpret_cast<const EpaLoopOutG<T>*>(rb->md);
    const uint32_t pair = rb->pair;
    const T r0 = swept_radius(lib.shapes[rb->sid1]), r1 = swept_radius(lib.shapes[rb->sid2]);
    EpaResult<T> res;
    res.status = lo->status;
    res.iterations = lo->iterations;
    res.normal = mk<T>(lo->nx, lo->ny, lo->nz);
    res.depth = lo->depth + (r0 + r1);
    res.rw0_ = mk<T>(lo->rw[0], lo->rw[1], lo->rw[2]);
    res.rw1_ = mk<T>(lo->rw[3], lo->rw[4], lo->rw[5]);
    res.rw2_ = mk<T>(lo->rw[6], lo->rw[7], lo->rw[8]);
    res.r00 = mk<T>(lo->r0[0], lo->r0[1], lo->r0[2]);
    res.r01 = mk<T>(lo->r0[3], lo->r0[4], lo->r0[5]);
    res.r02 = mk<T>(lo->r0[6], lo->r0[7], lo->r0[8]);
    PairOut<T> o;
    epa_finish(res, rb->gjk_iters, load_pose(io.tf1, pair), r0, r1, o);
    write_out<T>(io, q, pair, o);
    write_guess<T>(io, pair, o.cached_guess, 0, 0);
  }
}

#ifndef HFCL_EPA64_CURVED_WE
#define HFCL_EPA64_CURVED_WE 16
#endif
#ifndef HFCL_EPA_GRID_ROUNDS
#define HFCL_EPA_GRID_ROUNDS 2
#endif
template <class K>
static int resident_blocks_per_cu(K kernel) {
  int nb = 0;
  if (hipOccupancyMaxActiveBlocksPerMultiprocessor(&nb, reinterpret_cast<const void*>(kernel), 64, 0) != hipSuccess || nb < 1) nb = 8;
  hipFuncAttributes fa;
  if (hipFuncGetAttributes(&fa, reinterpret_cast<const void*>(kernel)) == hipSuccess && fa.sharedSizeBytes > 0) {
    const int units = int((fa.sharedSizeBytes + 1279) / 1280);
    nb = std::min(nb, 128 / units);
  }
  return std::max(nb, 1);
}
template <typename T>
void launch_epa_fast(int grid, hipStream_t st, const Work& wk, const LibView<T>& lv, const IO<T>& io, const QParams<T>& q, bool cc_queue, bool general_queue, int n_cus, bool curved_class, hipStream_t st2) {
  if constexpr (sizeof(T) == 4) {
    static const int per_cu_cc = resident_blocks_per_cu(k_epa_stream<T, EPA_WE, EPA_FAST_CAP, true>);
    static const int per_cu_gen = resident_blocks_per_cu(k_epa_stream<T, EPA_WE, EPA_FAST_CAP, false>);
    if (cc_queue)
      hipLaunchKernelGGL((k_epa_stream<T, EPA_WE, EPA_FAST_CAP, true>), dim3(std::min(grid, n_cus * per_cu_cc * HFCL_EPA_GRID_ROUNDS)), dim3(64), 0, st, wk, lv, io, q);
    if (general_queue)
      hipLaunchKernelGGL((k_epa_stream<T, EPA_WE, EPA_FAST_CAP, false>), dim3(std::min(grid, n_cus * per_cu_gen * HFCL_EPA_GRID_ROUNDS)), dim3(64), 0, st, wk, lv, io, q);
  } else {
#ifdef HFCL_EPA64_STREAM_CURVED
    static const int per_cu = resident_blocks_per_cu(k_epa_stream<T, HFCL_EPA64_CURVED_WE, epa_fast_cap<T>, false, true>);
    hipLaunchKernelGGL((k_epa_stream<T, HFCL_EPA64_CURVED_WE, epa_fast_cap<T>, false, true>), dim3(std::min(grid * (HFCL_EPA64_CURVED_WE / EPA_WE), n_cus * per_cu * HFCL_EPA_GRID_ROUNDS)), dim3(64), 0, st, wk, lv, io, q);
    hipLaunchKernelGGL((k_epa<T, EPA_WE, epa_small_cap<T>, 1, 1>), dim3(std::min(grid, n_cus * 32)), dim3(64), 0, st, wk, lv, io, q);
#else
    if (curved_class)
      hipLaunchKernelGGL((k_epa<T, HFCL_EPA64_CURVED_WE, epa_fast_cap<T>, 1, 2>), dim3(std::min(grid * (HFCL_EPA64_CURVED_WE / EPA_WE), n_cus * 16)), dim3(64), 0, st, wk, lv, io, q);
    hipLaunchKernelGGL((k_epa<T, EPA_WE, epa_small_cap<T>, 1, 1>), dim3(std::min(grid, n_cus * 32)), dim3(64), 0, (curved_class && st2) ? st2 : st, wk, lv, io, q);
#endif
  }
}
#if HFCL_UNIT_F32
template void launch_epa_fast<float>(int, hipStream_t, const Work&, const LibView<float>&, const IO<float>&, const QParams<float>&, bool, bool, int, bool, hipStream_t);
#endif
#if HFCL_UNIT_F64
template void launch_epa_fast<double>(int, hipStream_t, const Work&, const LibView<double>&, const IO<double>&, const QParams<double>&, bool, bool, int, bool, hipStream_t);
#endif

#if HFCL_UNIT_F32
void launch_epa_prepare(int grid, hipStream_t st, const Work& wk, const LibView<float>& lv, const IO<float>& io, const QParams<float>& q) {
  hipLaunchKernelGGL((k_epa_prepare<float>), dim3(grid), dim3(256), 0, st, wk, lv, io, q);
}
void launch_epa_loop(int grid, hipStream_t st, const Work& wk, const LibView<float>& lv, const QParams<float>& q, int n_cus) {
  static const int per_cu = resident_blocks_per_cu(k_epa_loop<float, EPA_WE, EPA_FAST_CAP>);
  hipLaunchKernelGGL((k_epa_loop<float, EPA_WE, EPA_FAST_CAP>), dim3(std::min(grid, n_cus * per_cu * HFCL_EPA_LOOP_ROUNDS)), dim3(64), 0, st, wk, lv, q);
}
void launch_epa_resume_cc(int grid, hipStream_t st, const Work& wk, const LibView<float>& lv, const IO<float>& io, const QParams<float>& q) {
  hipLaunchKernelGGL((k_epa_resume_cc<float, HFCL_EPA_CC_RESUME_WE>), dim3(grid), dim3(64), 0, st, wk, lv, io, q);
}
void launch_epa_records(int grid, hipStream_t st, const Work& wk, const LibView<float>& lv, const IO<float>& io, const QParams<float>& q) {
  hipLaunchKernelGGL((k_epa_records<float>), dim3(grid), dim3(256), 0, st, wk, lv, io, q);
}

#endif

#if !HFCL_KEEP_AB_FORMS
template <typename T> void launch_epa_prepare_general(int, hipStream_t, const Work&, const LibView<T>&, const IO<T>&, const QParams<T>&, bool) {}
template <typename T> void launch_epa_records_general(int, hipStream_t, const Work&, const LibView<T>&, const IO<T>&, const QParams<T>&, bool) {}
template <typename T> void launch_epa_loop_general(int, hipStream_t, hipStream_t, const Work&, const LibView<T>&, const QParams<T>&, int, bool) {}
#else
template <typename T>
void launch_epa_prepare_general(int grid, hipStream_t st, const Work& wk, const LibView<T>& lv, const IO<T>& io, const QParams<T>& q, bool skip_top) {
  hipLaunchKernelGGL((k_epa_prepare_general<T>), dim3(grid), dim3(256), 0, st, wk, lv, io, q, skip_top ? 1 : 0);
}
template <typename T>
void launch_epa_records_general(int grid, hipStream_t st, const Work& wk, const LibView<T>& lv, const IO<T>& io, const QParams<T>& q, bool skip_top) {
  hipLaunchKernelGGL((k_epa_records_general<T>), dim3(grid), dim3(256), 0, st, wk, lv, io, q, skip_top ? 1 : 0);
}
#ifndef HFCL_EPA_LOOPG_ROUNDS
#define HFCL_EPA_LOOPG_ROUNDS 1
#endif
template <typename T>
void launch_epa_loop_general(int grid, hipStream_t st, hipStream_t st2, const Work& wk, const LibView<T>& lv, const QParams<T>& q, int n_cus, bool curved_class) {
  if constexpr (sizeof(T) == 4) {
    static const int per_cu = resident_blocks_per_cu(k_epa_loop_general<T, EPA_WE, EPA_FAST_CAP, false>);
    hipLaunchKernelGGL((k_epa_loop_general<T, EPA_WE, EPA_FAST_CAP, false>), dim3(std::min(grid, n_cus * per_cu * HFCL_EPA_LOOPG_ROUNDS)), dim3(64), 0, st, wk, lv, q);
  } else {
    static const int per_cu_c = resident_blocks_per_cu(k_epa_loop_general<T, HFCL_EPA64_CURVED_WE, epa_fast_cap<T>, true>);
    static const int per_cu_p = resident_blocks_per_cu(k_epa_loop_general<T, EPA_WE, epa_small_cap<T>, false>);
    if (curved_class)
      hipLaunchKernelGGL((k_epa_loop_general<T, HFCL_EPA64_CURVED_WE, epa_fast_cap<T>, true>), dim3(std::min(grid * (HFCL_EPA64_CURVED_WE / EPA_WE), n_cus * per_cu_c * HFCL_EPA_LOOPG_ROUNDS)), dim3(64), 0, st, wk, lv, q);
    hipLaunchKernelGGL((k_epa_loop_general<T, EPA_WE, epa_small_cap<T>, false>), dim3(std::min(grid, n_cus * per_cu_p * HFCL_EPA_LOOPG_ROUNDS)), dim3(64), 0, (curved_class && st2) ? st2 : st, wk, lv, q);
  }
}
#endif
#define HFCL_INST_G(T)                                                                                                                                     \
  template void launch_epa_prepare_general<T>(int, hipStream_t, const Work&, const LibView<T>&, const IO<T>&, const QParams<T>&, bool);                   \
  template void launch_epa_records_general<T>(int, hipStream_t, const Work&, const LibView<T>&, const IO<T>&, const QParams<T>&, bool);                   \
  template void launch_epa_loop_general<T>(int, hipStream_t, hipStream_t, const Work&, const LibView<T>&, const QParams<T>&, int, bool);
#if HFCL_UNIT_F32
HFCL_INST_G(float)
#endif
#if HFCL_UNIT_F64
HFCL_INST_G(double)
#endif
#undef HFCL_INST_G

template <typename T>
void launch_epa_full(int grid, hipStream_t st, const Work& wk, const LibView<T>& lv, const IO<T>& io, const QParams<T>& q) {
  hipLaunchKernelGGL((k_epa<T, epa_we2<T>, EPA_MAX_ITER, 2>), dim3(grid), dim3(64), 0, st, wk, lv, io, q);
}
template <typename T>
__global__ void __launch_bounds__(1024) k_epa_requeue(Work wk) {
  __shared__ uint32_t base_s;
  const uint32_t n_bottom = min(wk.counts[B_COUNT], wk.n), n_top = min(wk.counts[B_COUNT + 3], wk.n - n_bottom);
  if (threadIdx.x == 0) base_s = wk.counts[B_COUNT + 1];
  __syncthreads();
  const uint32_t base = base_s;
  const EpaItem<T>* const src = reinterpret_cast<const EpaItem<T>*>(wk.epa_queue);
  EpaItem<T>* const dst = reinterpret_cast<EpaItem<T>*>(wk.epa_queue2);
  for (uint32_t i = threadIdx.x; i < n_bottom + n_top; i += blockDim.x) dst[base + i] = src[i < n_bottom ? i : wk.n - 1u - (i - n_bottom)];
  __syncthreads();
  if (threadIdx.x == 0) wk.counts[B_COUNT + 1] = base + n_bottom + n_top;
}
template <typename T>
void launch_epa_requeue(hipStream_t st, const Work& wk) {
  hipLaunchKernelGGL((k_epa_requeue<T>), dim3(1), dim3(1024), 0, st, wk);
}
#if HFCL_UNIT_F32
template void launch_epa_requeue<float>(hipStream_t, const Work&);
template void launch_epa_full<float>(int, hipStream_t, const Work&, const LibView<float>&, const IO<float>&, const QParams<float>&);
#endif
#if HFCL_UNIT_F64
template void launch_epa_requeue<double>(hipStream_t, const Work&);
template void launch_epa_full<double>(int, hipStream_t, const Work&, const LibView<double>&, const IO<double>&, const QParams<double>&);
#endif
```

### hpp-fcl_amd/csrc/hfcl_k_gjk.hip

```cpp
#include "hfcl_dev.hpp"
#include "hfcl_launch.hpp"

#ifndef HFCL_UNIT_PRECISION
#define HFCL_UNIT_PRECISION 0
#endif
#define HFCL_UNIT_F32 (HFCL_UNIT_PRECISION != 64)
#define HFCL_UNIT_F64 (HFCL_UNIT_PRECISION != 32)

#if HFCL_UNIT_F64
__global__ void __launch_bounds__(CLS_BLOCK) k_classify(Work wk, const uint8_t* kinds, uint32_t n_shapes, bool distance_mode) {
  constexpr int PER_THREAD = 8;
  constexpr uint32_t CHUNK = CLS_BLOCK * PER_THREAD;
  __shared__ uint32_t s_count[2 * B_COUNT];
  __shared__ uint32_t s_base[2 * B_COUNT];
  for (uint32_t start = blockIdx.x * CHUNK; start < wk.n; start += gridDim.x * CHUNK) {
    if (threadIdx.x < 2 * B_COUNT) s_count[threadIdx.x] = 0;
    __syncthreads();
    int bk[PER_THREAD];
    uint32_t rk[PER_THREAD];
#pragma unroll
    for (int k = 0; k < PER_THREAD; ++k) {
      const uint32_t i = start + k * CLS_BLOCK + threadIdx.x;
      bk[k] = -1;
      rk[k] = 0;
      if (i < wk.n) {
        const uint32_t s1 = wk.shape1[i], s2 = wk.shape2[i];
        if (s1 < n_shapes && s2 < n_shapes) {
          const int k1 = kinds[s1], k2 = kinds[s2];
          bk[k] = bucket_of(k1, k2, distance_mode);
          if ((bk[k] == B_PRIM || bk[k] == B_PC || bk[k] == B_CP) && curved_pair(k1, k2)) bk[k] += B_COUNT;
        } else {
          bk[k] = B_UNSUPPORTED;
        }
      }
      unsigned long long todo = __ballot(bk[k] >= 0);
      const int lane = threadIdx.x & 63;
      while (todo) {
        const int leader = __ffsll((long long)todo) - 1;
        const int c = __shfl(bk[k], leader, 64);
        const unsigned long long m = __ballot(bk[k] == c);
        uint32_t base = 0;
        if (lane == leader) base = atomicAdd(&s_count[c], (uint32_t)__popcll(m));
        base = __shfl(base, leader, 64);
        if (bk[k] == c) rk[k] = base + (uint32_t)__popcll(m & ((1ull << lane) - 1ull));
        todo &= ~m;
      }
    }
    __syncthreads();
    if (threadIdx.x < 2 * B_COUNT) {
      const uint32_t c = s_count[threadIdx.x];
      const int counter = threadIdx.x < B_COUNT ? int(threadIdx.x) : B_CURVED0 + int(threadIdx.x) - B_COUNT;
      s_base[threadIdx.x] = c ? atomicAdd(&wk.counts[counter], c) : 0u;
    }
    __syncthreads();
#pragma unroll
    for (int k = 0; k < PER_THREAD; ++k) {
      if (bk[k] < 0) continue;
      const uint32_t slot = s_base[bk[k]] + rk[k], id = start + k * CLS_BLOCK + threadIdx.x;
      if (bk[k] < B_COUNT)
        wk.lists[size_t(bk[k]) * wk.n + slot] = id;
      else
        wk.lists[size_t(bk[k] - B_COUNT) * wk.n + (wk.n - 1u - slot)] = id;
    }
    __syncthreads();
  }
}

#endif
template <typename T>
__global__ void __launch_bounds__(256) k_unsupported(Work wk, IO<T> io, int bucket) {
  const uint32_t cnt = wk.counts[bucket];
  for (uint32_t it = blockIdx.x * blockDim.x + threadIdx.x; it < cnt; it += gridDim.x * blockDim.x) {
    const uint32_t pair = wk.lists[size_t(bucket) * wk.n + it];
    auto r = io.out[pair];
    memset(&r, 0, sizeof(r));
    r.status = 0x80000000u;
    io.out[pair] = r;
  }
}

template <typename T>
__global__ void __launch_bounds__(256) k_closed(Work wk, LibView<T> lib, IO<T> io, QParams<T> q) {
  const uint32_t cnt = wk.counts[B_CLOSED];
  for (uint32_t it = blockIdx.x * blockDim.x + threadIdx.x; it < cnt; it += gridDim.x * blockDim.x) {
    const uint32_t pair = wk.lists[size_t(B_CLOSED) * wk.n + it];
    const DShape<T> a = lib.shapes[wk.shape1[pair]], b = lib.shapes[wk.shape2[pair]];
    const Pose<T> tf1 = load_pose(io.tf1, pair), tf2 = load_pose(io.tf2, pair);
    PairOut<T> o;
    o.distance = closed_form_distance(a, tf1, b, tf2, lib.verts, o.p1, o.p2, o.normal);
    o.gjk_status = GJK_DID_NOT_RUN;
    o.epa_status = EPA_DID_NOT_RUN;
    o.gjk_iters = o.epa_iters = 0;
    write_out<T>(io, q, pair, o);
    write_guess<T>(io, pair, initial_guess<T>(io, q, pair), 0, 0);
  }
}

#if HFCL_UNIT_F64
typedef double hfcl_d2 __attribute__((ext_vector_type(2)));
#ifndef HFCL_WPE_CLOSED
#define HFCL_WPE_CLOSED 2
#endif
__global__ void __launch_bounds__(256) __attribute__((amdgpu_waves_per_eu(HFCL_WPE_CLOSED, 8))) k_closed_staged(Work wk, LibView<double> lib, IO<double> io, QParams<double> q) {
  constexpr int NB = 256, PIECES = 6;
  __shared__ uint32_t s_pair[NB];
  __shared__ hfcl_d2 s_a[NB * PIECES];
  __shared__ hfcl_d2 s_b[NB * PIECES];
  static_assert(sizeof(hfcl_result) == 96, "record = 6 pieces");
  const uint32_t cnt = wk.counts[B_CLOSED];
  const uint32_t t = threadIdx.x;
  for (uint32_t base = blockIdx.x * NB; base < cnt; base += gridDim.x * NB) {
    const uint32_t nvalid = min(uint32_t(NB), cnt - base);
    s_pair[t] = wk.lists[size_t(B_CLOSED) * wk.n + base + (t < nvalid ? t : 0u)];
    __syncthreads();
#pragma unroll
    for (int j = 0; j < PIECES; ++j) {
      const uint32_t c = t + NB * j, p = c / PIECES, part = c % PIECES;
      const size_t pr = s_pair[p];
      s_a[c] = reinterpret_cast<const hfcl_d2*>(io.tf1 + 12 * pr)[part];
      s_b[c] = reinterpret_cast<const hfcl_d2*>(io.tf2 + 12 * pr)[part];
    }
    const uint32_t pair = s_pair[t];
    const DShape<double> a = lib.shapes[wk.shape1[pair]], b = lib.shapes[wk.shape2[pair]];
    __syncthreads();
    const Pose<double> tf1 = pose_from_abi<double>(reinterpret_cast<const double*>(s_a + PIECES * t));
    const Pose<double> tf2 = pose_from_abi<double>(reinterpret_cast<const double*>(s_b + PIECES * t));
    PairOut<double> o;
    o.distance = closed_form_distance(a, tf1, b, tf2, lib.verts, o.p1, o.p2, o.normal);
    o.gjk_status = GJK_DID_NOT_RUN;
    o.epa_status = EPA_DID_NOT_RUN;
    o.gjk_iters = o.epa_iters = 0;
    __syncthreads();
    IO<double> lio = io;
    lio.out = reinterpret_cast<hfcl_result*>(s_a);
    write_out<double>(lio, q, t, o);
    if (t < nvalid) write_guess<double>(io, pair, initial_guess<double>(io, q, pair), 0, 0);
    __syncthreads();
#pragma unroll
    for (int j = 0; j < PIECES; ++j) {
      const uint32_t c = t + NB * j, p = c / PIECES, part = c % PIECES;
      if (p < nvalid) reinterpret_cast<hfcl_d2*>(io.out + s_pair[p])[part] = s_a[c];
    }
    __syncthreads();
  }
}

#endif
template <typename T, class P, class PS>
__device__ __forceinline__ void finish_gjk(const Gjk<T, P>& g, const Work& wk, const IO<T>& io, const QParams<T>& q,
                                           uint32_t pair, const Pose<T>& tf1, T r0, T r1, const V3<T>& guess0,
                                           bool writer, const PS& ps, bool full_tier = false, bool cc_queue = false) {
  PairOut<T> o;
  EpaSeed<T> seed;
  const bool to_epa = gjk_finish(g, q, tf1, r0, r1, guess0, o, seed, ps);
  if (!writer) return;
  if (to_epa) {
    seed.pair = pair;
    if (cc_queue) {
#ifdef HFCL_EXPERIMENT_NO_QUEUE_ATOMIC
      const uint32_t slot = pair;
#else
// ... 39 lines not shown
    if constexpr (BVG)
      gjk_run(g, q.gjk, start_guess(q, a, b, sup.md, guess0), r0 + r1, false, sup, ps);
    else
      gjk_run(g, q.gjk, guess0, r0 + r1, false, sup, ps);
    finish_gjk<T>(g, wk, io, q, pair, tf1, r0, r1, guess0, true, ps, false, sizeof(T) == 8 && curved_pair(a.kind, b.kind));
  }
}
#ifndef HFCL_HULL_LDS_BATCH
#define HFCL_HULL_LDS_BATCH 4
#endif
template <typename T, int W, int NT>
struct HullLds {
  static constexpr int VPL = (HULL_MAX + W - 1) / W;
  static constexpr int WORDS = VPL * 3 * NT;
  T* lane;
  __device__ __forceinline__ void load(const T* verts, uint32_t n, int lig) {
#pragma unroll
    for (int k = 0; k < VPL; ++k) {
      uint32_t idx = uint32_t(lig * VPL + k);
      idx = idx < n ? idx : 0u;
      const T* p = verts + 3 * size_t(idx);
      lane[(3 * k + 0) * NT] = p[0];
      lane[(3 * k + 1) * NT] = p[1];
      lane[(3 * k + 2) * NT] = p[2];
    }
  }
  __device__ __forceinline__ V3<T> support(const V3<T>& dir, int lig) const {
#if HFCL_HULL_LDS_BATCH
    constexpr int B = HFCL_HULL_LDS_BATCH;
    T best = T(0);
    int bi = lig * VPL;
#pragma unroll
    for (int k0 = 0; k0 < VPL; k0 += B) {
      T vx[B], vy[B], vz[B];
#pragma unroll
      for (int j = 0; j < B; ++j) {
        vx[j] = lane[(3 * (k0 + j) + 0) * NT];
        vy[j] = lane[(3 * (k0 + j) + 1) * NT];
        vz[j] = lane[(3 * (k0 + j) + 2) * NT];
      }
      __builtin_amdgcn_sched_barrier(0);
#pragma unroll
      for (int j = 0; j < B; ++j) {
        const T d = vx[j] * dir.x + vy[j] * dir.y + vz[j] * dir.z;
        if (k0 + j == 0) {
          best = d;
        } else if (d > best) {
          best = d;
          bi = lig * VPL + k0 + j;
        }
      }
      __builtin_amdgcn_sched_barrier(0);
    }
#else
    T best = lane[0] * dir.x + lane[NT] * dir.y + lane[2 * NT] * dir.z;
    int bi = lig * VPL;
#pragma unroll
    for (int k = 1; k < VPL; ++k) {
      const T d = lane[(3 * k + 0) * NT] * dir.x + lane[(3 * k + 1) * NT] * dir.y + lane[(3 * k + 2) * NT] * dir.z;
      if (d > best) {
        best = d;
        bi = lig * VPL + k;
      }
    }
#endif
    butterfly_stages<W>([&](auto stage) {
      constexpr int M = decltype(stage)::value;
      const T od = group_exchange<W, M>(best);
      const int oi = group_exchange<W, M>(bi);
      const bool take = (od > best) | ((od == best) & (oi < bi));
      best = take ? od : best;
      bi = take ? oi : bi;
    });
    const int owner = bi / VPL, slot = bi % VPL;
    const T cx = lane[(3 * slot + 0) * NT], cy = lane[(3 * slot + 1) * NT], cz = lane[(3 * slot + 2) * NT];
    return mk<T>(__shfl(cx, owner, W), __shfl(cy, owner, W), __shfl(cz, owner, W));
  }
};
#ifndef HFCL_GJK_HULLB_LDS
#define HFCL_GJK_HULLB_LDS 1
#endif
template <typename T, int W, int M> constexpr bool hull_b_in_lds = HFCL_GJK_HULLB_LDS && M == 0 && W <= 4 && (HULL_MAX / W) * sizeof(T) <= 64;

template <typename T, int W, int M>
struct CvxSupport {
  DShape<T> a, b;
  HullRegs<T, W> h0;
  typename std::conditional<hull_b_in_lds<T, W, M>, HullLds<T, W, 256>, HullRegs<T, W>>::type h1;
  MDiff<T> md;
  int lig;
  __device__ __forceinline__ void eval(const V3<T>& dir, V3<T>& w, V3<T>& w0) const {
    if (M == 1)
      w0 = prim_support(a, dir);
    else
      w0 = h0.support(dir, lig);
    const V3<T> d1 = md.identity ? -dir : -tmul(md.oR1, dir);
    V3<T> s1;
    if (M == 2)
      s1 = prim_support(b, d1);
    else
      s1 = h1.support(d1, lig);
    s1 = md.identity ? s1 : (mul(md.oR1, s1) + md.ot1);
    w = w0 - s1;
  }
  __device__ __forceinline__ void operator()(const V3<T>& dir, V3<T>& w, V3<T>& w0) const { eval(dir, w, w0); }
};

template <typename T, int W, int M, bool BVG>
__device__ __forceinline__ void gjk_cvx_body(const Work& wk, const LibView<T>& lib, const IO<T>& io, const QParams<T>& q) {
  constexpr int BUCKET = (M == 0) ? B_CC : (M == 1 ? B_PC : B_CP);
  HFCL_GJK_W0_SLAB(T, 256, ps);
  __shared__ T hull_slab[hull_b_in_lds<T, W, M> ? HullLds<T, W, 256>::WORDS : 1];
  const BucketList list = bucket_list(wk, BUCKET);
  const int lig = threadIdx.x & (W - 1);
  const uint32_t groups = (gridDim.x * blockDim.x) / W;
  for (uint32_t it = (blockIdx.x * blockDim.x + threadIdx.x) / W; it < list.cnt; it += groups) {
    const uint32_t pair = list[it];
    CvxSupport<T, W, M> sup;
    if constexpr (hull_b_in_lds<T, W, M>) sup.h1.lane = hull_slab + threadIdx.x;
    sup.a = lib.shapes[wk.shape1[pair]];
    sup.b = lib.shapes[wk.shape2[pair]];
    sup.lig = lig;
    if (M != 1) sup.h0.load(lib.verts + 3 * size_t(sup.a.vertex_offset), sup.a.num_points, lig);
    if (M != 2) sup.h1.load(lib.verts + 3 * size_t(sup.b.vertex_offset), sup.b.num_points, lig);
    const Pose<T> tf1 = load_pose(io.tf1, pair), tf2 = load_pose(io.tf2, pair);
    sup.md = make_mdiff(tf1, tf2);
    const T r0 = swept_radius(sup.a), r1 = swept_radius(sup.b);
    const V3<T> guess0 = initial_guess<T>(io, q, pair);
    Gjk<T, typename GjkW0<T, 256>::P> g;
    if constexpr (BVG)
      gjk_run(g, q.gjk, start_guess(q, sup.a, sup.b, sup.md, guess0), r0 + r1, M == 0, sup, ps);
    else
      gjk_run(g, q.gjk, guess0, r0 + r1, M == 0, sup, ps);
    finish_gjk<T>(g, wk, io, q, pair, tf1, r0, r1, guess0, lig == 0, ps, false,
                  sizeof(T) == 4 ? M == 0 : (M != 0 && curved_pair(sup.a.kind, sup.b.kind)));
  }
}

template <int W, int M, bool BVG>
__global__ void __launch_bounds__(256) __attribute__((amdgpu_waves_per_eu(W == 2 ? HFCL_WPE_GJK_W2 : HFCL_WPE_GJK, 8)))
k_gjk_cvx(Work wk, LibView<float> lib, IO<float> io, QParams<float> q) {
  gjk_cvx_body<float, W, M, BVG>(wk, lib, io, q);
}
template <int W, int M, bool BVG>
__global__ void __launch_bounds__(256) __attribute__((amdgpu_waves_per_eu(HFCL_WPE_GJK64, 8)))
k_gjk_cvx64(Work wk, LibView<double> lib, IO<double> io, QParams<double> q) {
  gjk_cvx_body<double, W, M, BVG>(wk, lib, io, q);
}
template <int W, int M, bool BVG = false>
static void launch_gjk_cvx(int grid, hipStream_t st, const Work& wk, const LibView<float>& lv, const IO<float>& io, const QParams<float>& q) {
  hipLaunchKernelGGL((k_gjk_cvx<W, M, BVG>), dim3(grid), dim3(256), 0, st, wk, lv, io, q);
}
template <int W, int M, bool BVG = false>
static void launch_gjk_cvx(int grid, hipStream_t st, const Work& wk, const LibView<double>& lv, const IO<double>& io, const QParams<double>& q) {
  hipLaunchKernelGGL((k_gjk_cvx64<W, M, BVG>), dim3(grid), dim3(256), 0, st, wk, lv, io, q);
}
template <typename T>
struct LargeSupport {
  DShape<T> a, b;
  const T* va;
  const T* vb;
  HullGraph<T> ga, gb;
  mutable int hint0, hint1;
  MDiff<T> md;
  int lig;
  __device__ __forceinline__ V3<T> one(const DShape<T>& s, const T* v, const HullGraph<T>& g, const V3<T>& d, int& hint) const {
    return s.kind == K_CONVEX ? large_hull_support<T, LARGE_W>(v, s.num_points, g, d, lig, hint) : prim_support(s, d);
  }
  __device__ __forceinline__ void operator()(const V3<T>& dir, V3<T>& w, V3<T>& w0) const {
    w0 = one(a, va, ga, dir, hint0);
    const V3<T> d1 = md.identity ? -dir : -tmul(md.oR1, dir);
    V3<T> s1 = one(b, vb, gb, d1, hint1);
    s1 = md.identity ? s1 : (mul(md.oR1, s1) + md.ot1);
    w = w0 - s1;
  }
};

template <typename T, bool BVG>
__global__ void __launch_bounds__(256) __attribute__((amdgpu_waves_per_eu(2, 8))) k_gjk_large(Work wk, LibView<T> lib, IO<T> io, QParams<T> q) {
  HFCL_GJK_W0_SLAB(T, 256, ps);
  const uint32_t cnt = wk.counts[B_LARGE];
  const int lig = threadIdx.x & (LARGE_W - 1);
  const uint32_t groups = (gridDim.x * blockDim.x) / LARGE_W;
  for (uint32_t it = (blockIdx.x * blockDim.x + threadIdx.x) / LARGE_W; it < cnt; it += groups) {
    const uint32_t pair = wk.lists[size_t(B_LARGE) * wk.n + it];
    LargeSupport<T> sup;
    const uint32_t sid1 = wk.shape1[pair], sid2 = wk.shape2[pair];
    sup.a = lib.shapes[sid1];
    sup.b = lib.shapes[sid2];
    sup.va = lib.verts + 3 * size_t(sup.a.vertex_offset);
    sup.vb = lib.verts + 3 * size_t(sup.b.vertex_offset);
    sup.ga = sup.a.kind == K_CONVEX ? hull_graph(lib, sid1, sup.a.num_points) : HullGraph<T>{nullptr, nullptr};
    sup.gb = sup.b.kind == K_CONVEX ? hull_graph(lib, sid2, sup.b.num_points) : HullGraph<T>{nullptr, nullptr};
    sup.hint0 = sup.hint1 = -1;
    sup.lig = lig;
    const Pose<T> tf1 = load_pose(io.tf1, pair), tf2 = load_pose(io.tf2, pair);
    sup.md = make_mdiff(tf1, tf2);
    const T r0 = swept_radius(sup.a), r1 = swept_radius(sup.b);
    const V3<T> guess0 = initial_guess<T>(io, q, pair);
    Gjk<T, typename GjkW0<T, 256>::P> g;
    if constexpr (BVG)
      gjk_run(g, q.gjk, start_guess(q, sup.a, sup.b, sup.md, guess0), r0 + r1, sup.a.kind == K_CONVEX && sup.b.kind == K_CONVEX, sup, ps);
    else
      gjk_run(g, q.gjk, guess0, r0 + r1, sup.a.kind == K_CONVEX && sup.b.kind == K_CONVEX, sup, ps);
    finish_gjk<T>(g, wk, io, q, pair, tf1, r0, r1, guess0, lig == 0, ps, true);
  }
}

template <typename R>
__global__ void k_fill_skipped(R* out, uint32_t n) {
  for (uint32_t i = blockIdx.x * blockDim.x + threadIdx.x; i < n; i += gridDim.x * blockDim.x) {
    R r;
    memset(&r, 0, sizeof(r));
    r.distance = 3.402823466e+38f;
    r.status = 0x80000000u;
    out[i] = r;
  }
}
#if HFCL_UNIT_F64
template <>
__global__ void k_fill_skipped<hfcl_result>(hfcl_result* out, uint32_t n) {
  for (uint32_t i = blockIdx.x * blockDim.x + threadIdx.x; i < n; i += gridDim.x * blockDim.x) {
    hfcl_result r;
    const double x = __builtin_nan("");
    r.distance = 1.7976931348623157e+308;
    for (int k = 0; k < 3; ++k) r.normal[k] = r.p1[k] = r.p2[k] = x;
    r.b1 = r.b2 = -1;
    r.status = 0x80000000u;
    r.num_contacts = 0;
    out[i] = r;
  }
}

#endif
#if HFCL_UNIT_F64
__global__ void __launch_bounds__(256) k_expand_poses(const double* qt, double* tf, uint32_t n) {
  for (uint32_t i = blockIdx.x * blockDim.x + threadIdx.x; i < n; i += gridDim.x * blockDim.x) {
    const Pose<double> p = pose_from_quat<double, double>(qt + 7 * size_t(i));
    double* o = tf + 12 * size_t(i);
    o[0] = p.R.r0.x; o[1] = p.R.r1.x; o[2] = p.R.r2.x;
    o[3] = p.R.r0.y; o[4] = p.R.r1.y; o[5] = p.R.r2.y;
    o[6] = p.R.r0.z; o[7] = p.R.r1.z; o[8] = p.R.r2.z;
    o[9] = p.t.x; o[10] = p.t.y; o[11] = p.t.z;
  }
}
#endif
#if HFCL_UNIT_F64
void launch_expand_poses(hipStream_t st, const double* qt, double* tf, uint32_t n) {
  hipLaunchKernelGGL(k_expand_poses, dim3(1024), dim3(256), 0, st, qt, tf, n);
}
#endif

#if HFCL_UNIT_F64
void launch_classify(int grid, hipStream_t st, const Work& wk, const uint8_t* kinds, uint32_t n_shapes, bool distance_mode) {
  hipLaunchKernelGGL(k_classify, dim3(grid), dim3(CLS_BLOCK), 0, st, wk, kinds, n_shapes, distance_mode);
}
#endif
template <typename T>
void launch_unsupported(int grid, hipStream_t st, const Work& wk, const IO<T>& io, int bucket) {
  hipLaunchKernelGGL((k_unsupported<T>), dim3(grid), dim3(256), 0, st, wk, io, bucket);
}
#if HFCL_UNIT_F32
template void launch_unsupported<float>(int, hipStream_t, const Work&, const IO<float>&, int);
#endif
#if HFCL_UNIT_F64
template void launch_unsupported<double>(int, hipStream_t, const Work&, const IO<double>&, int);
#endif

template <typename T>
void launch_closed(int grid, hipStream_t st, const Work& wk, const LibView<T>& lv, const IO<T>& io, const QParams<T>& q, bool staged) {
#if HFCL_UNIT_F64
  if constexpr (sizeof(T) == 8) {
    if (staged) {
      hipLaunchKernelGGL(k_closed_staged, dim3(grid), dim3(256), 0, st, wk, lv, io, q);
      return;
    }
  }
#endif
  hipLaunchKernelGGL((k_closed<T>), dim3(grid), dim3(256), 0, st, wk, lv, io, q);
}
#if HFCL_UNIT_F32
template void launch_closed<float>(int, hipStream_t, const Work&, const LibView<float>&, const IO<float>&, const QParams<float>&, bool);
#endif
#if HFCL_UNIT_F64
template void launch_closed<double>(int, hipStream_t, const Work&, const LibView<double>&, const IO<double>&, const QParams<double>&, bool);
#endif

template <typename T>
void launch_gjk_prim(int grid, hipStream_t st, const Work& wk, const LibView<T>& lv, const IO<T>& io, const QParams<T>& q, bool bvg) {
  if (bvg)
    hipLaunchKernelGGL((k_gjk_prim<T, true>), dim3(grid), dim3(256), 0, st, wk, lv, io, q);
  else
    hipLaunchKernelGGL((k_gjk_prim<T, false>), dim3(grid), dim3(256), 0, st, wk, lv, io, q);
}
#if HFCL_UNIT_F32
template void launch_gjk_prim<float>(int, hipStream_t, const Work&, const LibView<float>&, const IO<float>&, const QParams<float>&, bool);
#endif
#if HFCL_UNIT_F64
template void launch_gjk_prim<double>(int, hipStream_t, const Work&, const LibView<double>&, const IO<double>&, const QParams<double>&, bool);
#endif

template <typename T, int M>
static void launch_gjk_cvx_m(int w, bool bvg, int grid, hipStream_t st, const Work& wk, const LibView<T>& lv, const IO<T>& io, const QParams<T>& q) {
  if (bvg) {
    if (w == 2) launch_gjk_cvx<2, M, true>(grid, st, wk, lv, io, q);
    else launch_gjk_cvx<4, M, true>(grid, st, wk, lv, io, q);
    return;
  }
  switch (w) {
    case 2: launch_gjk_cvx<2, M>(grid, st, wk, lv, io, q); break;
    case 8: launch_gjk_cvx<8, M>(grid, st, wk, lv, io, q); break;
    case 16: launch_gjk_cvx<16, M>(grid, st, wk, lv, io, q); break;
    case 32: launch_gjk_cvx<32, M>(grid, st, wk, lv, io, q); break;
    case 64: launch_gjk_cvx<64, M>(grid, st, wk, lv, io, q); break;
    default: launch_gjk_cvx<4, M>(grid, st, wk, lv, io, q); break;
  }
}
template <typename T>
void launch_gjk_cvx(int m, int w, bool bvg, int grid, hipStream_t st, const Work& wk, const LibView<T>& lv, const IO<T>& io, const QParams<T>& q) {
  if (m == 0) launch_gjk_cvx_m<T, 0>(w, bvg, grid, st, wk, lv, io, q);
  else if (m == 1) launch_gjk_cvx_m<T, 1>(w, bvg, grid, st, wk, lv, io, q);
  else launch_gjk_cvx_m<T, 2>(w, bvg, grid, st, wk, lv, io, q);
}
#if HFCL_UNIT_F32
template void launch_gjk_cvx<float>(int, int, bool, int, hipStream_t, const Work&, const LibView<float>&, const IO<float>&, const QParams<float>&);
#endif
#if HFCL_UNIT_F64
template void launch_gjk_cvx<double>(int, int, bool, int, hipStream_t, const Work&, const LibView<double>&, const IO<double>&, const QParams<double>&);
#endif

template <typename T>
void launch_gjk_large(int grid, hipStream_t st, const Work& wk, const LibView<T>& lv, const IO<T>& io, const QParams<T>& q, bool bvg) {
  if (bvg)
    hipLaunchKernelGGL((k_gjk_large<T, true>), dim3(grid), dim3(256), 0, st, wk, lv, io, q);
  else
    hipLaunchKernelGGL((k_gjk_large<T, false>), dim3(grid), dim3(256), 0, st, wk, lv, io, q);
}
#if HFCL_UNIT_F32
template void launch_gjk_large<float>(int, hipStream_t, const Work&, const LibView<float>&, const IO<float>&, const QParams<float>&, bool);
#endif
#if HFCL_UNIT_F64
template void launch_gjk_large<double>(int, hipStream_t, const Work&, const LibView<double>&, const IO<double>&, const QParams<double>&, bool);
#endif

#if HFCL_UNIT_F64
void launch_fill_skipped(hipStream_t st, hfcl_result* out, uint32_t n) {
  hipLaunchKernelGGL((k_fill_skipped<hfcl_result>), dim3(1024), dim3(256), 0, st, out, n);
}
#endif
// ... 6 lines not shown
```

### hpp-fcl_amd/csrc/hfcl_launch.hpp

```cpp
#pragma once
#include "hfcl_dev.hpp"

void launch_classify(int grid, hipStream_t st, const Work& wk, const uint8_t* kinds, uint32_t n_shapes, bool distance_mode);
template <typename T> void launch_unsupported(int grid, hipStream_t st, const Work& wk, const IO<T>& io, int bucket);
template <typename T> void launch_closed(int grid, hipStream_t st, const Work& wk, const LibView<T>& lv, const IO<T>& io, const QParams<T>& q, bool staged);
template <typename T> void launch_gjk_prim(int grid, hipStream_t st, const Work& wk, const LibView<T>& lv, const IO<T>& io, const QParams<T>& q, bool bvg);
template <typename T> void launch_gjk_cvx(int m, int w, bool bvg, int grid, hipStream_t st, const Work& wk, const LibView<T>& lv, const IO<T>& io, const QParams<T>& q);
template <typename T> void launch_gjk_large(int grid, hipStream_t st, const Work& wk, const LibView<T>& lv, const IO<T>& io, const QParams<T>& q, bool bvg);
void launch_expand_poses(hipStream_t st, const double* qt, double* tf, uint32_t n);
void launch_fill_skipped(hipStream_t st, hfcl_result* out, uint32_t n);
void launch_fill_skipped(hipStream_t st, hfcl_result_f32* out, uint32_t n);
void launch_compact_records(hipStream_t st, const hfcl_result* in, hfcl_result_compact* out, uint32_t n);
void launch_compact_records(hipStream_t st, const hfcl_result_f32* in, hfcl_result_compact_f32* out, uint32_t n);

template <typename T> void launch_epa_fast(int grid, hipStream_t st, const Work& wk, const LibView<T>& lv, const IO<T>& io, const QParams<T>& q, bool cc_queue, bool general_queue, int n_cus, bool curved_class = true, hipStream_t st2 = nullptr);
void launch_epa_prepare(int grid, hipStream_t st, const Work& wk, const LibView<float>& lv, const IO<float>& io, const QParams<float>& q);
void launch_epa_loop(int grid, hipStream_t st, const Work& wk, const LibView<float>& lv, const QParams<float>& q, int n_cus);
void launch_epa_resume_cc(int grid, hipStream_t st, const Work& wk, const LibView<float>& lv, const IO<float>& io, const QParams<float>& q);
void launch_epa_records(int grid, hipStream_t st, const Work& wk, const LibView<float>& lv, const IO<float>& io, const QParams<float>& q);
template <typename T> void launch_epa_prepare_general(int grid, hipStream_t st, const Work& wk, const LibView<T>& lv, const IO<T>& io, const QParams<T>& q, bool skip_top);
template <typename T> void launch_epa_loop_general(int grid, hipStream_t st, hipStream_t st2, const Work& wk, const LibView<T>& lv, const QParams<T>& q, int n_cus, bool curved_class);
template <typename T> void launch_epa_records_general(int grid, hipStream_t st, const Work& wk, const LibView<T>& lv, const IO<T>& io, const QParams<T>& q, bool skip_top);
template <typename T> void launch_epa_requeue(hipStream_t st, const Work& wk);
template <typename T> void launch_epa_full(int grid, hipStream_t st, const Work& wk, const LibView<T>& lv, const IO<T>& io, const QParams<T>& q);

struct AsideStream {
  hipStream_t stream;
  hipEvent_t fork, join;
};
template <typename T> void launch_bvh_collide(int grid, hipStream_t st, const Work& wk, const LibView<T>& lv, const BvhView<T>& bv, const IO<T>& io, const QParams<T>& q, const BvhParams& bp, T break_distance2, BvhSplit split, BvhSpill spill, const AsideStream* aside = nullptr);
template <typename T> void launch_bvh_distance(int grid, hipStream_t st, const Work& wk, const LibView<T>& lv, const BvhView<T>& bv, const IO<T>& io, const QParams<T>& q, BvhSpill spill);
template <typename T> void launch_bvh_shape(int grid, hipStream_t st, const Work& wk, const LibView<T>& lv, const BvhView<T>& bv, const IO<T>& io, const QParams<T>& q, const BvhParams& bp, T break_distance2);
template <typename T> void launch_bvh_shape_distance_fast(int grid, int grid_finish, hipStream_t st, const Work& wk, const LibView<T>& lv, const BvhView<T>& bv, const IO<T>& io, const QParams<T>& q, BvhSpill spill);
template <typename T> void launch_bvh_shape_fast(int grid, int grid_finish, int coop_grid, hipStream_t st, const Work& wk, const LibView<T>& lv, const BvhView<T>& bv, const IO<T>& io, const QParams<T>& q, const BvhParams& bp, T break_distance2, BvhSplit split, BvhSpill spill, const AsideStream* aside = nullptr);
template <typename T> void launch_bvh_shape_distance(int grid, hipStream_t st, const Work& wk, const LibView<T>& lv, const BvhView<T>& bv, const IO<T>& io, const QParams<T>& q);
template <typename T> void launch_triangle(int grid, hipStream_t st, const Work& wk, const LibView<T>& lv, const IO<T>& io, const QParams<T>& q);

struct PatchArgs {
  const uint32_t* s1;
  const uint32_t* s2;
  const double* tf1;
  const double* tf2;
  const hfcl_result* rec;
  const hfcl_guess* guess;
  uint32_t n, n_shapes;
  const DShape<double>* shapes;
  const double* verts;
  const uint32_t* graph_base;
  const uint32_t* graph_off;
  const uint32_t* graph_ent;
  uint32_t max_num_patch, num_samples;
  double tol;
  uint32_t pcap, plim;
  hfcl_contact_patch* out;
  double* out_pts;
  uint32_t* lists;
  uint32_t* counts;
  char* ws;
  size_t slot_bytes;
  uint32_t nslots, cap, cloud_cap, vis_cap;
};
void launch_patch(hipStream_t st, const PatchArgs& a, int max_blocks, const char** names, hipEvent_t* e0, hipEvent_t* e1);

struct SceneExpandArgs {
  const uint32_t* pairs;
  const uint32_t* object_shape;
  const void* object_tf;
  uint64_t n_objects;
  uint32_t n_pairs;
  uint64_t q0;
  uint64_t c0;
  uint32_t p0;
  uint32_t m;
  uint32_t* s1;
  uint32_t* s2;
  void* tf1;
  void* tf2;
};
void launch_scene_expand(hipStream_t st, const SceneExpandArgs& a, bool f32, int max_blocks);
struct SceneFoldArgs {
  const void* rec;
  uint64_t q0, q1;
  uint32_t n_pairs;
  uint64_t g0;
  uint64_t n_pieces;
  double margin;
  int collide;
  hfcl_scene_summary* summary;
  hfcl_scene_summary* partials;
};
void launch_scene_fold(hipStream_t st, const SceneFoldArgs& a, bool f32, int max_blocks);
```

Before: 604.1 million queries/s.

## Fuse counter readback and reset into last-block kernel, add EPA tickets and GJK block knob

The per-batch counter memset and device-to-host memcpy are replaced. The unsupported kernel now runs once over a bitmask of buckets, and its last finishing block writes the counters into mapped coherent host memory and zeroes them for the next batch. The mesh-beside heuristic reads the host counters only after an event reports them complete. An optional ticket-based work-stealing tail for the f32 EPA loop (off by default) and a configurable block size for f32 convex GJK are also added. This cuts two stream operations per batch, at the cost of a grid-wide atomic and a system-scope fence in the last block.

```diff
diff --git a/hpp-fcl_amd/csrc/hfcl_dev.hpp b/hpp-fcl_amd/csrc/hfcl_dev.hpp
--- a/hpp-fcl_amd/csrc/hfcl_dev.hpp
+++ b/hpp-fcl_amd/csrc/hfcl_dev.hpp
@@ -46,6 +46,7 @@
 constexpr int CTR_SHAPE_DEFER_MARK = 2 * B_COUNT + 13;
 constexpr int CTR_DIST_RERUN = 2 * B_COUNT + 14, CTR_SHAPE_DIST_RERUN = 2 * B_COUNT + 15;
 constexpr int N_COUNTERS = 2 * B_COUNT + 16;
+constexpr int COUNTS_WORDS = N_COUNTERS + 1;
 
 constexpr int K_CONVEX_LARGE = 21;
 
@@ -148,7 +149,9 @@
   void* epa_ready_g;
   uint32_t* epa_cc_over;
   uint32_t cc_resume_base, cc_resume_cap;
-};
+  uint32_t* epa_tickets;
+};
+constexpr int EPA_TICKET_TEAMS = 64, EPA_TICKET_STRIDE = 32;
 __host__ __device__ inline bool curved_pair(int k1, int k2) {
   return k1 == K_ELLIPSOID || k1 == K_CONE || k1 == K_CYLINDER || k2 == K_ELLIPSOID || k2 == K_CONE || k2 == K_CYLINDER;
 }
diff --git a/hpp-fcl_amd/csrc/hfcl_host.hip b/hpp-fcl_amd/csrc/hfcl_host.hip
--- a/hpp-fcl_amd/csrc/hfcl_host.hip
+++ b/hpp-fcl_amd/csrc/hfcl_host.hip
@@ -27,6 +27,11 @@
       return HFCL_ERR_HIP;                                                                    \
     }                                                                                         \
   } while (0)
+
+#ifndef HFCL_EPA_LOOP_TICKETS_DEFAULT
+#define HFCL_EPA_LOOP_TICKETS_DEFAULT 0
+#endif
+constexpr unsigned COUNTS_HOST_FLAGS = hipHostMallocMapped | hipHostMallocCoherent;
 
 struct KernelTime {
   const char* name;
@@ -59,14 +64,20 @@
   size_t epa_capacity = 0;
   uint32_t* d_lists = nullptr;
   uint32_t* d_counts = nullptr;
+  bool counts_clean = false;
+  bool counts_memset = false;
   void* d_epa_queue = nullptr;
   void* d_epa_queue2 = nullptr;
   uint32_t* d_epa_cc_over = nullptr;
+  uint32_t* d_epa_tickets = nullptr;
+  uint32_t epa_loop_tickets = HFCL_EPA_LOOP_TICKETS_DEFAULT;
   hipStream_t aux = nullptr;
   hipStream_t mesh_st = nullptr;
   hipEvent_t ev_mesh_fork = nullptr, ev_mesh_join = nullptr;
   hipStream_t mesh_st2 = nullptr, mesh_aux = nullptr;
   bool ran_batch = false;
+  hipEvent_t ev_counts = nullptr;
+  bool beside_last = true;
   hipEvent_t ev_mesh_fork2 = nullptr, ev_mesh_join2 = nullptr;
   BvhTask* d_bvh2_tasks = nullptr;
   void* d_bvh2_sums = nullptr;
@@ -453,7 +464,7 @@
       "bvh_walk_rounds", "bvh_walk_order", "mesh_beside", "mesh_prio", "shape_walk", "shape_walk_sort", "shape_walk_budget", "shape_walk_min", "gjk_beside_max", "epa_direct_max", "bvh_walk_k", "bvh_walk_budget", "shape_dist_leaf_min", "shape_dist_starve", "bvhd_leaf_min", "bvhd_starve",
       "bvhd_part_min", "shape_dist_budget", "bvh_budget0_coop", "shape_budget0", "shape_budget", "shape_leaf_cost", "shape_levels",
       "climb_min", "bvh_budget", "bvh_budget0", "bvh_levels", "cvx_w", "epa_resume_slots", "bvh_task_slots", "bvh_force_wide",
-      "pipe_trace", "scene_chunk", nullptr};
+      "pipe_trace", "scene_chunk", "epa_loop_tickets", "counts_memset", nullptr};
   return keys;
 }
 static int parse_list(const char* v, uint32_t* out, int first, int cap, uint32_t lo, uint32_t hi) {
@@ -483,6 +494,8 @@
   else if (key == "epa_general_staged_min") lib->epa_general_staged_min = size_t(std::max(0ll, i));
   else if (key == "epa64_two_streams") lib->epa64_two_streams = on;
   else if (key == "epa_cc_staged_min") lib->epa_cc_staged_min = size_t(std::max(0ll, i));
+  else if (key == "counts_memset") lib->counts_memset = on;
+  else if (key == "epa_loop_tickets") lib->epa_loop_tickets = uint32_t(std::min(std::max(0ll, i), 100ll));
   else if (key == "pipe_chunk") lib->pipe_chunk = strtoull(v, nullptr, 10);
   else if (key == "bvh_filter") {
     if (on && !HFCL_KEEP_AB_FORMS) return HFCL_ERR_INVALID_ARGUMENT;
@@ -548,8 +561,11 @@
   hfcl_lib* lib = new hfcl_lib();
   lib->device = device;
   bool ok = upload_shapes(lib, shapes, n_shapes, vertices, n_vertices);
-  ok = ok && hipMalloc(&lib->d_counts, N_COUNTERS * sizeof(uint32_t)) == hipSuccess;
-  ok = ok && hipHostMalloc((void**)&lib->h_counts, N_COUNTERS * sizeof(uint32_t), hipHostMallocDefault) == hipSuccess;
+  ok = ok && hipMalloc(&lib->d_counts, COUNTS_WORDS * sizeof(uint32_t)) == hipSuccess;
+  ok = ok && hipMemset(lib->d_counts, 0, COUNTS_WORDS * sizeof(uint32_t)) == hipSuccess;
+  lib->counts_clean = ok;
+  ok = ok && hipMalloc(&lib->d_epa_tickets, size_t(EPA_TICKET_TEAMS) * EPA_TICKET_STRIDE * sizeof(uint32_t)) == hipSuccess;
+  ok = ok && hipHostMalloc((void**)&lib->h_counts, N_COUNTERS * sizeof(uint32_t), COUNTS_HOST_FLAGS) == hipSuccess;
   if (ok) memset(lib->h_counts, 0, N_COUNTERS * sizeof(uint32_t));
   if (!ok) {
     set_error("hfcl_lib_create: HIP allocation/copy failed");
@@ -593,6 +609,8 @@
     hipFree(lib->d_graph_ent64);
   }
   hipFree(lib->d_counts);
+  hipFree(lib->d_epa_tickets);
+  if (lib->ev_counts) hipEventDestroy(lib->ev_counts);
   if (lib->h_counts) hipHostFree(lib->h_counts);
   hipFree(lib->d_patch_ws);
   hipFree(lib->d_patch_lists);
@@ -1311,6 +1329,7 @@
   wk.epa_ready = nullptr;
   wk.epa_ready_g = nullptr;
   wk.epa_cc_over = lib->d_epa_cc_over;
+  wk.epa_tickets = lib->d_epa_tickets;
   wk.cc_resume_base = wk.resume_cap;
   {
     const size_t fslots = lib->resume_cap * std::max(epa_resume_stride<double>, epa_resume_stride<float>) / epa_resume_stride<float>;
@@ -1347,7 +1366,8 @@
   auto may = [&](int b) { return (lib->possible_buckets >> b) & 1u; };
   const bool any_gjk = may(B_PRIM) || may(B_CC) || may(B_PC) || may(B_CP) || may(B_LARGE);
   const bool bvg = q.guess_mode == HFCL_GUESS_BOUNDING_VOLUME;
-  HIP_TRY(hipMemsetAsync(lib->d_counts, 0, N_COUNTERS * sizeof(uint32_t), st));
+  if (!lib->counts_clean || lib->counts_memset) HIP_TRY(hipMemsetAsync(lib->d_counts, 0, COUNTS_WORDS * sizeof(uint32_t), st));
+  lib->counts_clean = false;
   tbeg("k_classify");
   launch_classify(blocks_for(n, CLS_BLOCK * 8), st, wk, lib->d_kinds, uint32_t(lib->n_shapes), q.mode != 1);
   tend();
@@ -1408,6 +1428,7 @@
     return HFCL_OK;
   };
   bool meshes_on_own_stream = false;
+  bool mixed_library = false;
   auto launch_meshes = [&]() -> int {
     if (!lib->h_meshes.empty() && (may(B_BVH) || may(B_BVHSHAPE))) {
       const hfcl_lib* owner = lib;
@@ -1660,10 +1681,14 @@
     const bool any_mesh = !lib->h_meshes.empty() && (may(B_BVH) || may(B_BVHSHAPE));
     const bool any_solid = may(B_CLOSED) || any_gjk || may(B_TRI);
     bool beside = any_mesh && any_solid && lib->mesh_beside;
+    mixed_library = beside;
     if (beside && lib->mesh_beside < 4 && lib->ran_batch && lib->h_counts) {
-      uint32_t solids_before = 0, meshes_before = one_count(lib->h_counts, int(B_BVH)) + one_count(lib->h_counts, int(B_BVHSHAPE));
-      for (int b : {int(B_CLOSED), int(B_PRIM), int(B_CC), int(B_PC), int(B_CP), int(B_LARGE), int(B_TRI)}) solids_before += one_count(lib->h_counts, b);
-      if (!solids_before || !meshes_before) beside = false;
+      if (lib->ev_counts && hipEventQuery(lib->ev_counts) == hipSuccess) {
+        uint32_t solids_before = 0, meshes_before = one_count(lib->h_counts, int(B_BVH)) + one_count(lib->h_counts, int(B_BVHSHAPE));
+        for (int b : {int(B_CLOSED), int(B_PRIM), int(B_CC), int(B_PC), int(B_CP), int(B_LARGE), int(B_TRI)}) solids_before += one_count(lib->h_counts, b);
+        lib->beside_last = solids_before && meshes_before;
+      }
+      if (!lib->beside_last) beside = false;
     }
     if (beside && ensure_mesh_stream(lib) != HFCL_OK) beside = false;
     if (beside) {
@@ -1755,7 +1780,7 @@
       }
     }
     if constexpr (F32) {
-      if (cc_staged) launch_epa_loop(epa_batches, st, wk, lv, q, lib->n_cus);
+      if (cc_staged) launch_epa_loop(epa_batches, st, wk, lv, q, lib->n_cus, lib->epa_loop_tickets);
     }
     if (gen_staged) launch_epa_loop_general<T>(epa_batches, st, st2, wk, lv, q, lib->n_cus, lib->has_curved);
     if ((F32 && may(B_CC) && !cc_staged) || (general_q && !gen_staged))
@@ -1801,15 +1826,20 @@
   }
   if (mesh_join_pending) HIP_TRY(hipStreamWaitEvent(st, lib->ev_mesh_join, 0));
   tbeg("k_unsupported");
-  if (may(B_UNSUPPORTED)) launch_unsupported<T>(blocks_for(n, 256 * 64), st, wk, io, int(B_UNSUPPORTED));
+  uint32_t flag = may(B_UNSUPPORTED) ? 1u << B_UNSUPPORTED : 0u;
   if (lib->h_meshes.empty()) {
-    if (may(B_BVHSHAPE)) launch_unsupported<T>(blocks_for(n, 256 * 64), st, wk, io, int(B_BVHSHAPE));
-    if (may(B_BVH)) launch_unsupported<T>(blocks_for(n, 256 * 64), st, wk, io, int(B_BVH));
-  }
+    if (may(B_BVHSHAPE)) flag |= 1u << B_BVHSHAPE;
+    if (may(B_BVH)) flag |= 1u << B_BVH;
+  }
+  launch_unsupported<T>(flag ? blocks_for(n, 256 * 64) : 1, st, wk, io, flag, lib->counts_dst ? lib->counts_dst : lib->h_counts);
   tend();
-  HIP_TRY(hipMemcpyAsync(lib->counts_dst ? lib->counts_dst : lib->h_counts, lib->d_counts, N_COUNTERS * sizeof(uint32_t), hipMemcpyDeviceToHost, st));
+  HIP_TRY(hipGetLastError());
+  lib->counts_clean = true;
   lib->ran_batch = lib->counts_dst == nullptr;
-  HIP_TRY(hipGetLastError());
+  if (lib->ran_batch && mixed_library) {
+    if (!lib->ev_counts) HIP_TRY(hipEventCreateWithFlags(&lib->ev_counts, hipEventDisableTiming));
+    HIP_TRY(hipEventRecord(lib->ev_counts, st));
+  }
   return HFCL_OK;
 }
 
@@ -1846,9 +1876,14 @@
   h->epa_general_staged_min = lib->epa_general_staged_min;
   h->epa64_two_streams = lib->epa64_two_streams;
   h->epa_cc_staged_min = lib->epa_cc_staged_min;
+  h->epa_loop_tickets = lib->epa_loop_tickets;
+  h->counts_memset = lib->counts_memset;
   h->n_cus = lib->n_cus;
-  bool ok = hipMalloc(&h->d_counts, N_COUNTERS * sizeof(uint32_t)) == hipSuccess;
-  ok = ok && hipHostMalloc((void**)&h->h_counts, N_COUNTERS * sizeof(uint32_t), hipHostMallocDefault) == hipSuccess;
+  bool ok = hipMalloc(&h->d_counts, COUNTS_WORDS * sizeof(uint32_t)) == hipSuccess;
+  ok = ok && hipMemset(h->d_counts, 0, COUNTS_WORDS * sizeof(uint32_t)) == hipSuccess;
+  h->counts_clean = ok;
+  ok = ok && hipMalloc(&h->d_epa_tickets, size_t(EPA_TICKET_TEAMS) * EPA_TICKET_STRIDE * sizeof(uint32_t)) == hipSuccess;
+  ok = ok && hipHostMalloc((void**)&h->h_counts, N_COUNTERS * sizeof(uint32_t), COUNTS_HOST_FLAGS) == hipSuccess;
   ok = ok && hipMalloc(&h->d_epa_v0, size_t(h->n_cus) * 16 * (64 / EPA_WE2) * EPA_MAX_VERTS * sizeof(Quad<double>)) == hipSuccess;
   if (!ok) {
     hfcl_lib_destroy(h);
@@ -2075,8 +2110,8 @@
       HIP_TRY(hipEventCreateWithFlags(&sg.ev_in, hipEventDisableTiming));
       HIP_TRY(hipEventCreateWithFlags(&sg.ev_done, hipEventDisableTiming));
       HIP_TRY(hipEventCreateWithFlags(&sg.ev_in2, hipEventDisableTiming));
-      HIP_TRY(hipHostMalloc((void**)&sg.h_counts, N_COUNTERS * sizeof(uint32_t), hipHostMallocDefault));
-      HIP_TRY(hipHostMalloc((void**)&sg.h_counts2, N_COUNTERS * sizeof(uint32_t), hipHostMallocDefault));
+      HIP_TRY(hipHostMalloc((void**)&sg.h_counts, N_COUNTERS * sizeof(uint32_t), COUNTS_HOST_FLAGS));
+      HIP_TRY(hipHostMalloc((void**)&sg.h_counts2, N_COUNTERS * sizeof(uint32_t), COUNTS_HOST_FLAGS));
     }
   }
   if (n > lib->st_capacity) {
@@ -2166,7 +2201,7 @@
   if (!lib->d_pack) {
     const size_t cap = up(C * (2 * 96 + sizeof(hfcl_guess)) + 2 * up(C * 4)) + up(C * (sizeof(hfcl_result) + sizeof(hfcl_guess))) + 2 * C * 96 + 1024;
     HIP_TRY(hipHostMalloc((void**)&lib->h_pack, cap, hipHostMallocDefault));
-    HIP_TRY(hipHostMalloc((void**)&lib->h_pack_counts, 2 * N_COUNTERS * sizeof(uint32_t), hipHostMallocDefault));
+    HIP_TRY(hipHostMalloc((void**)&lib->h_pack_counts, 2 * N_COUNTERS * sizeof(uint32_t), COUNTS_HOST_FLAGS));
     HIP_TRY(hipMalloc(&lib->d_pack, cap));
   }
   if (!lib->s_cmp) {
@@ -3206,7 +3241,7 @@
   }
   constexpr int CS = hfcl_lib::SceneWs::COUNT_SLOTS;
   constexpr size_t SLOT_WORDS = 2 * size_t(N_COUNTERS);
-  if (!w.h_counts) HIP_TRY(hipHostMalloc((void**)&w.h_counts, CS * SLOT_WORDS * sizeof(uint32_t), hipHostMallocDefault));
+  if (!w.h_counts) HIP_TRY(hipHostMalloc((void**)&w.h_counts, CS * SLOT_WORDS * sizeof(uint32_t), COUNTS_HOST_FLAGS));
   for (hipEvent_t& e : w.ev_counts)
     if (!e) HIP_TRY(hipEventCreateWithFlags(&e, hipEventDisableTiming));
   memset(w.h_counts, 0, CS * SLOT_WORDS * sizeof(uint32_t));
diff --git a/hpp-fcl_amd/csrc/hfcl_k_epa.hip b/hpp-fcl_amd/csrc/hfcl_k_epa.hip
--- a/hpp-fcl_amd/csrc/hfcl_k_epa.hip
+++ b/hpp-fcl_amd/csrc/hfcl_k_epa.hip
@@ -282,6 +282,7 @@
   const uint32_t cnt = wk.counts[B_COUNT + 3];
   const EpaItem<T>* const queue = reinterpret_cast<const EpaItem<T>*>(wk.epa_queue);
   EpaReady<T>* const ready = reinterpret_cast<EpaReady<T>*>(wk.epa_ready);
+  if (wk.epa_tickets && blockIdx.x == 0 && threadIdx.x < EPA_TICKET_TEAMS) wk.epa_tickets[threadIdx.x * EPA_TICKET_STRIDE] = 0u;
   for (uint32_t i = blockIdx.x * blockDim.x + threadIdx.x; i < cnt; i += gridDim.x * blockDim.x) {
     bool live = false;
     EpaReady<T> rb;
@@ -348,7 +349,7 @@
 }
 template <typename T, int WE, int CAP>
 __global__ void __launch_bounds__(64) __attribute__((amdgpu_waves_per_eu(HFCL_WPE_EPA32_CC, 8)))
-k_epa_loop(Work wk, LibView<T> lib, QParams<T> q) {
+k_epa_loop(Work wk, LibView<T> lib, QParams<T> q, uint32_t ticket_pct) {
   constexpr int G = 64 / WE;
   static_assert(WE >= 8, "a group's lanes copy the eight records of a block");
   typedef LaneGroup<WE> Grp;
@@ -361,6 +362,10 @@
   int state = IDLE;
   uint32_t it = 0;
   uint32_t next = blockIdx.x;
+  const uint32_t pool0 = ticket_pct ? uint32_t(uint64_t(cnt) * (100u - ticket_pct) / (100ull * gridDim.x)) * gridDim.x : cnt;
+  const uint32_t n_teams = min(uint32_t(EPA_TICKET_TEAMS), gridDim.x);
+  const uint32_t team = blockIdx.x % n_teams;
+  bool pool_empty = ticket_pct == 0u;
   EpaSupportCC<T, WE> sup;
   sup.lig = lig;
   Epa<T, Grp, CAP, V0_TAG> epa;
@@ -368,8 +373,14 @@
   while (true) {
     const uint64_t live = __ballot(state == LIVE);
     const int n_live = __popcll(live) / WE;
-    const bool more = next < cnt;
+    const bool more = next < pool0 || !pool_empty;
     if (n_live == 0 || (more && G - n_live >= HFCL_EPA_LOOP_REFILL_MIN)) {
+      const uint32_t n_idle = uint32_t(G - n_live);
+      uint32_t n_own = 0;
+      while (n_own < n_idle && next + n_own * gridDim.x < pool0) ++n_own;
+      const uint32_t n_claim = pool_empty ? 0u : n_idle - n_own;
+      uint32_t ticket = 0;
+      if (n_claim && lane == 0) ticket = atomicAdd(&wk.epa_tickets[team * EPA_TICKET_STRIDE], n_claim);
       if (state != LIVE) {
         if (state != IDLE) {
           EpaReady<T>* rb = ready + it;
@@ -401,9 +412,18 @@
           Grp::sync();
           state = IDLE;
         }
+      }
+      uint64_t claimed = 0;
+      if (n_claim) {
+        claimed = uint64_t(pool0) + team + uint64_t(__builtin_amdgcn_readfirstlane(ticket)) * n_teams;
+        pool_empty = claimed + uint64_t(n_claim) * n_teams >= cnt;
+      }
+      if (state != LIVE) {
         const uint64_t lower = live | ~((uint64_t(1) << (grp * WE)) - 1);
         const uint32_t rank = uint32_t(__popcll(~lower)) / WE;
-        it = next + rank * gridDim.x;
+        const uint64_t it64 = rank < n_own ? uint64_t(next) + uint64_t(rank) * gridDim.x
+                                           : (n_claim ? claimed + uint64_t(rank - n_own) * n_teams : uint64_t(cnt));
+        it = uint32_t(it64 < cnt ? it64 : cnt);
         if (it < cnt) {
           const EpaReady<T>* rb = ready + it;
           const uint32_t packed = rb->packed;
@@ -421,8 +441,8 @@
           }
         }
       }
-      next += uint32_t(G - n_live) * gridDim.x;
-      if (n_live == 0 && !more) {
+      next += n_own * gridDim.x;
+      if (n_live == 0 && !(next < pool0 || !pool_empty)) {
         if (__ballot(state == LIVE) == 0) break;
       }
       continue;
@@ -731,9 +751,10 @@
 void launch_epa_prepare(int grid, hipStream_t st, const Work& wk, const LibView<float>& lv, const IO<float>& io, const QParams<float>& q) {
   hipLaunchKernelGGL((k_epa_prepare<float>), dim3(grid), dim3(256), 0, st, wk, lv, io, q);
 }
-void launch_epa_loop(int grid, hipStream_t st, const Work& wk, const LibView<float>& lv, const QParams<float>& q, int n_cus) {
+void launch_epa_loop(int grid, hipStream_t st, const Work& wk, const LibView<float>& lv, const QParams<float>& q, int n_cus, uint32_t ticket_pct) {
   static const int per_cu = resident_blocks_per_cu(k_epa_loop<float, EPA_WE, EPA_FAST_CAP>);
-  hipLaunchKernelGGL((k_epa_loop<float, EPA_WE, EPA_FAST_CAP>), dim3(std::min(grid, n_cus * per_cu * HFCL_EPA_LOOP_ROUNDS)), dim3(64), 0, st, wk, lv, q);
+  hipLaunchKernelGGL((k_epa_loop<float, EPA_WE, EPA_FAST_CAP>), dim3(std::min(grid, n_cus * per_cu * HFCL_EPA_LOOP_ROUNDS)), dim3(64), 0, st, wk, lv, q,
+                     wk.epa_tickets ? ticket_pct : 0u);
 }
 void launch_epa_resume_cc(int grid, hipStream_t st, const Work& wk, const LibView<float>& lv, const IO<float>& io, const QParams<float>& q) {
   hipLaunchKernelGGL((k_epa_resume_cc<float, HFCL_EPA_CC_RESUME_WE>), dim3(grid), dim3(64), 0, st, wk, lv, io, q);
diff --git a/hpp-fcl_amd/csrc/hfcl_k_gjk.hip b/hpp-fcl_amd/csrc/hfcl_k_gjk.hip
--- a/hpp-fcl_amd/csrc/hfcl_k_gjk.hip
+++ b/hpp-fcl_amd/csrc/hfcl_k_gjk.hip
@@ -68,15 +68,33 @@
 
 #endif
 template <typename T>
-__global__ void __launch_bounds__(256) k_unsupported(Work wk, IO<T> io, int bucket) {
-  const uint32_t cnt = wk.counts[bucket];
-  for (uint32_t it = blockIdx.x * blockDim.x + threadIdx.x; it < cnt; it += gridDim.x * blockDim.x) {
-    const uint32_t pair = wk.lists[size_t(bucket) * wk.n + it];
-    auto r = io.out[pair];
-    memset(&r, 0, sizeof(r));
-    r.status = 0x80000000u;
-    io.out[pair] = r;
-  }
+__global__ void __launch_bounds__(256) k_unsupported(Work wk, IO<T> io, uint32_t buckets, uint32_t* host_counts) {
+  for (int bucket = 0; bucket < B_COUNT; ++bucket) {
+    if (!((buckets >> bucket) & 1u)) continue;
+    const uint32_t cnt = wk.counts[bucket];
+    for (uint32_t it = blockIdx.x * blockDim.x + threadIdx.x; it < cnt; it += gridDim.x * blockDim.x) {
+      const uint32_t pair = wk.lists[size_t(bucket) * wk.n + it];
+      auto r = io.out[pair];
+      memset(&r, 0, sizeof(r));
+      r.status = 0x80000000u;
+      io.out[pair] = r;
+    }
+  }
+  __shared__ uint32_t s_last;
+  __syncthreads();
+  if (threadIdx.x == 0) {
+    __threadfence();
+    s_last = atomicAdd(&wk.counts[N_COUNTERS], 1u) == gridDim.x - 1u;
+  }
+  __syncthreads();
+  if (!s_last) return;
+  if (threadIdx.x < N_COUNTERS) {
+    const uint32_t c = __hip_atomic_load(&wk.counts[threadIdx.x], __ATOMIC_RELAXED, __HIP_MEMORY_SCOPE_AGENT);
+    __hip_atomic_store(&host_counts[threadIdx.x], c, __ATOMIC_RELAXED, __HIP_MEMORY_SCOPE_SYSTEM);
+    wk.counts[threadIdx.x] = 0u;
+  }
+  if (threadIdx.x == N_COUNTERS) wk.counts[N_COUNTERS] = 0u;
+  __threadfence_system();
 }
 
 template <typename T>
@@ -282,11 +300,15 @@
 #endif
 template <typename T, int W, int M> constexpr bool hull_b_in_lds = HFCL_GJK_HULLB_LDS && M == 0 && W <= 4 && (HULL_MAX / W) * sizeof(T) <= 64;
 
-template <typename T, int W, int M>
+#ifndef HFCL_GJK_CC_WG
+#define HFCL_GJK_CC_WG 256
+#endif
+template <typename T, int W, int M> constexpr int cvx_block = (sizeof(T) == 4 && W == 2 && M == 0) ? HFCL_GJK_CC_WG : 256;
+template <typename T, int W, int M, int NT = cvx_block<T, W, M>>
 struct CvxSupport {
   DShape<T> a, b;
   HullRegs<T, W> h0;
-  typename std::conditional<hull_b_in_lds<T, W, M>, HullLds<T, W, 256>, HullRegs<T, W>>::type h1;
+  typename std::conditional<hull_b_in_lds<T, W, M>, HullLds<T, W, NT>, HullRegs<T, W>>::type h1;
   MDiff<T> md;
   int lig;
   __device__ __forceinline__ void eval(const V3<T>& dir, V3<T>& w, V3<T>& w0) const {
@@ -309,14 +331,15 @@
 template <typename T, int W, int M, bool BVG>
 __device__ __forceinline__ void gjk_cvx_body(const Work& wk, const LibView<T>& lib, const IO<T>& io, const QParams<T>& q) {
   constexpr int BUCKET = (M == 0) ? B_CC : (M == 1 ? B_PC : B_CP);
-  HFCL_GJK_W0_SLAB(T, 256, ps);
-  __shared__ T hull_slab[hull_b_in_lds<T, W, M> ? HullLds<T, W, 256>::WORDS : 1];
+  constexpr int NT = cvx_block<T, W, M>;
+  HFCL_GJK_W0_SLAB(T, NT, ps);
+  __shared__ T hull_slab[hull_b_in_lds<T, W, M> ? HullLds<T, W, NT>::WORDS : 1];
   const BucketList list = bucket_list(wk, BUCKET);
   const int lig = threadIdx.x & (W - 1);
   const uint32_t groups = (gridDim.x * blockDim.x) / W;
   for (uint32_t it = (blockIdx.x * blockDim.x + threadIdx.x) / W; it < list.cnt; it += groups) {
     const uint32_t pair = list[it];
-    CvxSupport<T, W, M> sup;
+    CvxSupport<T, W, M, NT> sup;
     if constexpr (hull_b_in_lds<T, W, M>) sup.h1.lane = hull_slab + threadIdx.x;
     sup.a = lib.shapes[wk.shape1[pair]];
     sup.b = lib.shapes[wk.shape2[pair]];
@@ -327,7 +350,7 @@
     sup.md = make_mdiff(tf1, tf2);
     const T r0 = swept_radius(sup.a), r1 = swept_radius(sup.b);
     const V3<T> guess0 = initial_guess<T>(io, q, pair);
-    Gjk<T, typename GjkW0<T, 256>::P> g;
+    Gjk<T, typename GjkW0<T, NT>::P> g;
     if constexpr (BVG)
       gjk_run(g, q.gjk, start_guess(q, sup.a, sup.b, sup.md, guess0), r0 + r1, M == 0, sup, ps);
     else
@@ -338,7 +361,7 @@
 }
 
 template <int W, int M, bool BVG>
-__global__ void __launch_bounds__(256) __attribute__((amdgpu_waves_per_eu(W == 2 ? HFCL_WPE_GJK_W2 : HFCL_WPE_GJK, 8)))
+__global__ void __launch_bounds__((cvx_block<float, W, M>)) __attribute__((amdgpu_waves_per_eu(W == 2 ? HFCL_WPE_GJK_W2 : HFCL_WPE_GJK, 8)))
 k_gjk_cvx(Work wk, LibView<float> lib, IO<float> io, QParams<float> q) {
   gjk_cvx_body<float, W, M, BVG>(wk, lib, io, q);
 }
@@ -349,7 +372,8 @@
 }
 template <int W, int M, bool BVG = false>
 static void launch_gjk_cvx(int grid, hipStream_t st, const Work& wk, const LibView<float>& lv, const IO<float>& io, const QParams<float>& q) {
-  hipLaunchKernelGGL((k_gjk_cvx<W, M, BVG>), dim3(grid), dim3(256), 0, st, wk, lv, io, q);
+  constexpr int NT = cvx_block<float, W, M>;
+  hipLaunchKernelGGL((k_gjk_cvx<W, M, BVG>), dim3(grid * (256 / NT)), dim3(NT), 0, st, wk, lv, io, q);
 }
 template <int W, int M, bool BVG = false>
 static void launch_gjk_cvx(int grid, hipStream_t st, const Work& wk, const LibView<double>& lv, const IO<double>& io, const QParams<double>& q) {
@@ -457,14 +481,14 @@
 }
 #endif
 template <typename T>
-void launch_unsupported(int grid, hipStream_t st, const Work& wk, const IO<T>& io, int bucket) {
-  hipLaunchKernelGGL((k_unsupported<T>), dim3(grid), dim3(256), 0, st, wk, io, bucket);
+void launch_unsupported(int grid, hipStream_t st, const Work& wk, const IO<T>& io, uint32_t buckets, uint32_t* host_counts) {
+  hipLaunchKernelGGL((k_unsupported<T>), dim3(grid), dim3(256), 0, st, wk, io, buckets, host_counts);
 }
 #if HFCL_UNIT_F32
-template void launch_unsupported<float>(int, hipStream_t, const Work&, const IO<float>&, int);
-#endif
-#if HFCL_UNIT_F64
-template void launch_unsupported<double>(int, hipStream_t, const Work&, const IO<double>&, int);
+template void launch_unsupported<float>(int, hipStream_t, const Work&, const IO<float>&, uint32_t, uint32_t*);
+#endif
+#if HFCL_UNIT_F64
+template void launch_unsupported<double>(int, hipStream_t, const Work&, const IO<double>&, uint32_t, uint32_t*);
 #endif
 
 template <typename T>
diff --git a/hpp-fcl_amd/csrc/hfcl_launch.hpp b/hpp-fcl_amd/csrc/hfcl_launch.hpp
--- a/hpp-fcl_amd/csrc/hfcl_launch.hpp
+++ b/hpp-fcl_amd/csrc/hfcl_launch.hpp
@@ -2,7 +2,7 @@
 #include "hfcl_dev.hpp"
 
 void launch_classify(int grid, hipStream_t st, const Work& wk, const uint8_t* kinds, uint32_t n_shapes, bool distance_mode);
-template <typename T> void launch_unsupported(int grid, hipStream_t st, const Work& wk, const IO<T>& io, int bucket);
+template <typename T> void launch_unsupported(int grid, hipStream_t st, const Work& wk, const IO<T>& io, uint32_t buckets, uint32_t* host_counts);
 template <typename T> void launch_closed(int grid, hipStream_t st, const Work& wk, const LibView<T>& lv, const IO<T>& io, const QParams<T>& q, bool staged);
 template <typename T> void launch_gjk_prim(int grid, hipStream_t st, const Work& wk, const LibView<T>& lv, const IO<T>& io, const QParams<T>& q, bool bvg);
 template <typename T> void launch_gjk_cvx(int m, int w, bool bvg, int grid, hipStream_t st, const Work& wk, const LibView<T>& lv, const IO<T>& io, const QParams<T>& q);
@@ -15,7 +15,7 @@
 
 template <typename T> void launch_epa_fast(int grid, hipStream_t st, const Work& wk, const LibView<T>& lv, const IO<T>& io, const QParams<T>& q, bool cc_queue, bool general_queue, int n_cus, bool curved_class = true, hipStream_t st2 = nullptr);
 void launch_epa_prepare(int grid, hipStream_t st, const Work& wk, const LibView<float>& lv, const IO<float>& io, const QParams<float>& q);
-void launch_epa_loop(int grid, hipStream_t st, const Work& wk, const LibView<float>& lv, const QParams<float>& q, int n_cus);
+void launch_epa_loop(int grid, hipStream_t st, const Work& wk, const LibView<float>& lv, const QParams<float>& q, int n_cus, uint32_t ticket_pct);
 void launch_epa_resume_cc(int grid, hipStream_t st, const Work& wk, const LibView<float>& lv, const IO<float>& io, const QParams<float>& q);
 void launch_epa_records(int grid, hipStream_t st, const Work& wk, const LibView<float>& lv, const IO<float>& io, const QParams<float>& q);
 template <typename T> void launch_epa_prepare_general(int grid, hipStream_t st, const Work& wk, const LibView<T>& lv, const IO<T>& io, const QParams<T>& q, bool skip_top);
```

Measured after the change: 598.3 million queries/s. About the same (-1.0%).
